# Charrrrrlie/X-as-Supervision

Hardware: AMD Instinct MI355X
Metric: images/sec HM36_Multi_SurS1 256px bs32 (full disc+gen training step) (higher is better)
Workload: dtype f32 (f16x3 split: every fp32 operand as two fp16 pieces, three products; f32 accumulate); 1 GPU; HM36_Multi_SurS1; batch_per_gpu=32, cameras=4, image=256x256, parallelism=dp1, ranks=1, precision=f16x3, dedupe=False, full=False

## Files before the change

include/xas_hip.h:

```cpp
#ifndef XAS_HIP_H
#define XAS_HIP_H

#include <stddef.h>
#include <stdint.h>

#ifdef __cplusplus
extern "C" {
#endif

const char* xas_last_error(void);
enum {
  XAS_TUNE_WGRAD_SPLIT_XCD = 1,
  XAS_TUNE_PLAIN_KLOOP = 32,
  XAS_TUNE_GLOBAL_LOAD = 64,
  XAS_TUNE_WGRAD_GLOBAL_LOAD = 128,
  XAS_TUNE_WGRAD_ALT_ORDER = 8192,
  XAS_TUNE_WGRAD_PLAIN_KLOOP = 524288,
  XAS_TUNE_SLAB_SHIFT = 15,
  XAS_TUNE_SLAB_MASK = 3,
  XAS_TUNE_SLAB_512 = 32768,
  XAS_TUNE_SLAB_128 = 65536,
  XAS_TUNE_SLAB_64 = 98304,
  XAS_TUNE_COL_REDUCE_LEAN = 262144,
  XAS_TUNE_GENERAL_KERNELS = 1 << 22,
  XAS_TUNE_NO_WIDE_TILES = 1 << 23,
  XAS_TUNE_NO_STEM_WGRAD = 1 << 24,
  XAS_TUNE_STEM_FWD_F32 = 1 << 25,
  XAS_TUNE_NO_X6P = 1 << 26,
  XAS_TUNE_X6P_ANY_K = 1 << 27
};
int xas_set_tuning(int flags);
enum { XAS_PREC_F32 = 0, XAS_PREC_BF16 = 1, XAS_PREC_BF16X6 = 2, XAS_PREC_F16X3 = 3 };
#define XAS_AMAX_SUB 32
#define XAS_AMAX_STRIDE 32
#define XAS_AMAX_SLOT_FLOATS (XAS_AMAX_SUB * XAS_AMAX_STRIDE)
enum { XAS_GRAD_IS_X = 0x100 };
int xas_set_precision(int mode);
int xas_get_precision(void);
int xas_abi_version(void);

#define XAS_HEAD_STATS 16
size_t xas_head_workspace_floats(int B, int K, int D);
int xas_head_softargmax_fwd(const float* logits, int B, int K, int D, int num_hypo, int neighbor,
                            float* kps, int64_t* z_idx, float* depth_prob_map, int groups, float* stats,
                            float* partial, void* stream);
int xas_head_softargmax_from_partials(const float* partial, int B, int K, int D, int nchunk, int num_hypo, int neighbor,
                                      float* kps, int64_t* z_idx, float* depth_prob_map, int groups, float* stats,
                                      void* stream);
int xas_head_softargmax_flip_from_partials(const float* partial, int B, int K, int D, int nchunk, int num_hypo, int neighbor,
                                           const int* perm, float* kps, int64_t* z_idx, float* depth_prob_map, int groups,
                                           void* stream);
int xas_head_softargmax_fwd_flip(const float* logits, int B, int K, int D, int num_hypo, int neighbor, const int* perm,
                                 float* kps, int64_t* z_idx, float* depth_prob_map, int groups, float* partial, void* stream);

int xas_head_softargmax_bwd(const float* logits, const float* stats, const int64_t* z_idx,
                            const float* grad_kps, int B, int K, int D, int num_hypo, int neighbor,
                            float* grad_logits, float* coef, void* stream);
int xas_head_softargmax_bwd_amax(const float* logits, const float* stats, const int64_t* z_idx,
                                 const float* grad_kps, int B, int K, int D, int num_hypo, int neighbor,
                                 float* grad_logits, float* coef, float* amax_out, void* stream);

#define XAS_HEAD_SPREAD 5
size_t xas_head_spread_workspace_floats(int B, int K, int D);
int xas_head_spread(const float* logits, int B, int K, int D, float* spread , float* workspace, void* stream);

#define XAS_GEO_NORM 1
#define XAS_GEO_MONO 2
#define XAS_GEO_PATCH 4
#define XAS_GEO_IMAGE 8
int xas_patch_to_world_fwd(const float* kps, const float* trans_image, const float* k_mat,
                           const float* pelvis, const float* rot_world, const float* trans_world,
                           int B, int Hy, int K, float image_size, float rect_width, int flags,
                           float* world, void* stream);
int xas_patch_to_world_bwd(const float* kps, const float* grad_world, const float* trans_image,
                           const float* k_mat, const float* pelvis, const float* rot_world,
                           const float* trans_world, int B, int Hy, int K, float image_size,
                           float rect_width, int flags, float* grad_kps, void* stream);

#define XAS_GEO_WORLD 16
int xas_world_to_patch_fwd(const float* pts, const float* pre_rot, float pre_scale, int pelvis_origin,
                           const float* trans_image, const float* k_mat, const float* pelvis,
                           const float* rot_world, const float* trans_world, int B, int Hy, int K,
                           float image_size, float rect_width, int flags, float* out, void* stream);
int xas_world_to_patch_bwd(const float* pts, const float* grad_out, const float* pre_rot, float pre_scale,
                           int pelvis_origin, const float* trans_image, const float* k_mat, const float* pelvis,
                           const float* rot_world, const float* trans_world, int B, int Hy, int K,
                           float image_size, float rect_width, int flags, float* grad_pts, float* grad_pre_rot,
                           void* stream);

int xas_lines_nblk(int S);
int xas_draw_lines_max_fwd(const float* kps, long kp_stride_b, long kp_stride_j, int B, int K,
                           const int* parents, const int* children, int L, unsigned fine_mask,
                           float body_width, int S, float* mask, void* stream);
int xas_draw_lines_max_bwd(const float* kps, long kp_stride_b, long kp_stride_j, int B, int K,
                           const int* parents, const int* children, int L, unsigned fine_mask,
                           float body_width, int S, const float* grad_mask, float* partial,
                           float* grad_kps_xy , void* stream);

typedef struct {
  int N, Hi, Wi, Cin;
  int Cout, R, S;
  int stride, pad;
  int Ho, Wo;
  int mode;
  const float* grad_amax;
  const float* x_amax;
} xas_conv_shape;

int xas_conv_weight_planes(const xas_conv_shape* s, int pass);
int xas_conv_kernel_class(const xas_conv_shape* s, int pass);
int xas_f16_weight_overflow(int reset);
int xas_f16_weight_overflow_peek(unsigned* device_out, void* stream);
size_t xas_split_weight_bytes(long rows, long K, int pieces);
int xas_split_weight(const float* w_packed, void* w_split, long rows, long K, int pieces, void* stream);

int xas_prepare_weights(const void* descs, int n, long blocks, void* stream);

int xas_conv_fwd(const float* x, const float* w_packed, const float* bias, float* y,
                 const xas_conv_shape* s, void* stream);

int xas_conv_fwd_head_chunks(const xas_conv_shape* s, int K, int D);
int xas_conv_fwd_head(const float* x, const float* w_packed, const float* bias, float* y, const xas_conv_shape* s,
                      int K, int D, float* head_partial, void* stream);
size_t xas_conv_fwd_bnstats_workspace_floats(const xas_conv_shape* s, int groups);
int xas_conv_fwd_bnstats(const float* x, const float* w_packed, float* y, const xas_conv_shape* s, int groups,
                         const float* pivot, float* mean, float* var_biased, long out_stride, float* count_out,
                         float* workspace, float* running_mean, float* running_var, float momentum, void* stream);
size_t xas_conv_dgrad_bn_bwd_workspace_floats(const xas_conv_shape* s, int groups);
int xas_conv_dgrad_bn_bwd(const float* dy, const float* w_packed_t, const xas_conv_shape* s, const float* xb,
                          const float* mean, const float* var_biased, const float* gamma, const float* beta, float eps,
                          int groups, double count, float* dz, float* dx, float* sums, float* workspace, float* dbeta_acc,
                          float* dgamma_acc, void* stream);
int xas_conv_dgrad(const float* dy, const float* w_packed_t, float* dx,
                   const xas_conv_shape* s, void* stream);
int xas_conv_dgrad_acc(const float* dy, const float* w_packed_t, float* dx, const xas_conv_shape* shape, void* stream);
int xas_conv_dgrad_acc_masked(const float* dy, const float* w_packed_t, float* dx, const xas_conv_shape* s,
                              const float* dprev, const uint8_t* mask, void* stream);
enum {
  XAS_PLAN_ROUTE = 0,
  XAS_PLAN_KERNEL = 1,
  XAS_PLAN_BM = 2,
  XAS_PLAN_BN = 3,
  XAS_PLAN_PIPELINED = 4,
  XAS_PLAN_PHASES = 5,
  XAS_PLAN_PIECES = 6,
  XAS_PLAN_PATCH_WIDTH = 7,
  XAS_PLAN_TPB = 8,
  XAS_PLAN_IMAGES = 9,
  XAS_PLAN_INTS = 10
};
enum { XAS_ROUTE_STEM_F16 = 1, XAS_ROUTE_STEM_F32 = 2, XAS_ROUTE_THIN_VEC_TO_SCALAR = 3, XAS_ROUTE_THIN_SCALAR_TO_VEC = 4,
       XAS_ROUTE_DIRECT = 5, XAS_ROUTE_MFMA = 6 };
enum { XAS_KERNEL_IGEMM_BUF = 1, XAS_KERNEL_IGEMM = 2, XAS_KERNEL_IGEMM_X6 = 3, XAS_KERNEL_IGEMM_X6T = 4, XAS_KERNEL_IGEMM_X6P = 5 };
int xas_conv_igemm_plan(const xas_conv_shape* s, int pass, int has_bias, int* out);
size_t xas_conv_wgrad_workspace_floats(const xas_conv_shape* s);
int xas_conv_wgrad(const float* x, const float* dy, float* dw_packed, float* workspace,
                   const xas_conv_shape* s, void* stream);
int xas_conv_wgrad_oihw(const float* x, const float* dy, float* dw_oihw, float* workspace,
                        const xas_conv_shape* s, void* stream);
int xas_conv_wgrad_acc(const float* x, const float* dy, float* dw_oihw, float* workspace,
                       const xas_conv_shape* s, void* stream);
int xas_pack_weight(const float* oihw, float* packed, int Cout, int Cin, int R, int S,
                    int transposed, void* stream);
int xas_unpack_weight(const float* packed, float* oihw, int Cout, int Cin, int R, int S,
                      int transposed, void* stream);

size_t xas_bn_workspace_floats(long M, int C, int groups);
int xas_bn_stats(const float* x, long M, int C, int groups, float* mean, float* var_biased, long out_stride,
                 float* count_out, float* workspace, float* running_mean, float* running_var, float momentum,
                 long count, void* stream);
int xas_bn_stats_from_partials(const float* partial, long rows, int C, int groups, long rows_per_group,
                               const float* pivot, float* mean, float* var_biased, long out_stride, float* count_out,
                               float* workspace, float* running_mean, float* running_var, float momentum, void* stream);
int xas_bn_bwd_sums_from_partials(const float* partial, long rows, int C, int groups, float* sums, float* workspace,
                                  float* dbeta_acc, float* dgamma_acc, void* stream);
int xas_bn_sync_merge(const float* gathered, int world, int groups, int C, long msg_stride, float* mean,
                      float* var_biased, float* running_mean, float* running_var, float momentum, void* stream);
int xas_col_sum(const float* x, long M, int C, float* out, float* workspace, void* stream);
int xas_col_sum_acc(const float* x, long M, int C, float* acc, float* workspace, void* stream);
int xas_bn_apply(const float* x, const float* mean, const float* var_biased, const float* gamma,
                 const float* beta, const float* residual, float eps, int act, long M, int C, int groups,
                 float* y, uint8_t* mask_out, void* stream);
int xas_bn_apply_amax(const float* x, const float* mean, const float* var_biased, const float* gamma,
                      const float* beta, const float* residual, float eps, int act, long M, int C, int groups,
                      float* y, uint8_t* mask_out, float* amax_out, void* stream);
int xas_abs_max(const float* x, long n, float* amax_out, void* stream);
int xas_bn_update_running(const float* mean, const float* var_biased, float* running_mean,
                          float* running_var, float momentum, long count, int C, int groups, void* stream);
int xas_bn_bwd_reduce(const float* x, const float* y, const float* dy, const float* mean,
                      const float* var_biased, const float* gamma, const float* beta, float eps, int act,
// ... 130 lines not shown
```

x-as-supervision_amd/csrc/bn.hip:

```cpp
#include "common.h"

namespace xas {


struct ColGeom { int TX, TY, CB, ncb, nslab, G; long rows_per_slab, Mg; };

static int col_geom(long M, int C, int G, ColGeom* g) {
  XAS_REQUIRE(M > 0 && C >= 4 && C % 4 == 0, "column reduce: channel count %d must be a positive multiple of 4", C);
  XAS_REQUIRE(G >= 1 && G <= 64 && M % G == 0, "column reduce: %ld rows do not split into %d equal groups", M, G);
  int cb = 4;
  while (cb < 64 && C % (cb * 2) == 0) cb *= 2;
  g->CB = cb; g->G = G; g->Mg = M / G;
  g->TX = g->CB / 4; g->TY = 256 / g->TX; g->ncb = C / g->CB;
  static const long kWant[4] = {256, 512, 128, 64};
  long want = kWant[(tune_flags() >> XAS_TUNE_SLAB_SHIFT) & XAS_TUNE_SLAB_MASK] * (G > 1 ? 2 : 1) / ((long)g->ncb * G);
  long maxslab = cdiv(g->Mg, (long)g->TY * 8);
  if (want > maxslab) want = maxslab;
  if (want < 1) want = 1;
  g->rows_per_slab = cdiv(g->Mg, want);
  g->nslab = (int)cdiv(g->Mg, g->rows_per_slab);
  return 0;
}

constexpr int kTicketWords = 65536;
// ... 687 lines not shown
      const int wo = e / C4, c = (e - wo * C4) * 4;
      float4 best = make_float4(-INFINITY, -INFINITY, -INFINITY, -INFINITY);
      int b0 = 0, b1 = 0, b2 = 0, b3 = 0;
      bool first = true;
#pragma unroll
      for (int r = 0; r < 3; ++r) {
        const int hi = ho * 2 - 1 + r;
        if ((unsigned)hi >= (unsigned)H) continue;
#pragma unroll
        for (int s = 0; s < 3; ++s) {
          const int wi = wo * 2 - 1 + s;
          if ((unsigned)wi >= (unsigned)W) continue;
          const float4 v = *reinterpret_cast<const float4*>(xn + ((size_t)hi * W + wi) * C + c);
          const int tap = r * 3 + s;
          if (first || v.x > best.x) { best.x = v.x; b0 = tap; }
          if (first || v.y > best.y) { best.y = v.y; b1 = tap; }
          if (first || v.z > best.z) { best.z = v.z; b2 = tap; }
          if (first || v.w > best.w) { best.w = v.w; b3 = tap; }
          first = false;
        }
      }
      *reinterpret_cast<float4*>(y + (obase + e) * 4) = best;
      *reinterpret_cast<char4*>(idx + (obase + e) * 4) = make_char4((char)b0, (char)b1, (char)b2, (char)b3);
    }
  }
}

__global__ __launch_bounds__(256) void maxpool_bwd_kernel(const float* __restrict__ dy, const int8_t* __restrict__ idx, int N, int H,
                                                          int W, int C, int Ho, int Wo, float* __restrict__ dx) {
  const int C4 = C / 4, per_row = W * C4;
  for (int row = blockIdx.x; row < N * H; row += gridDim.x) {
    const int n = row / H, hi = row - n * H;
    const size_t obase = (size_t)row * per_row;
    for (int e = threadIdx.x; e < per_row; e += blockDim.x) {
      const int wi = e / C4, c = (e - wi * C4) * 4;
      float4 acc = make_float4(0, 0, 0, 0);
      for (int ho = hi / 2; ho <= (hi + 1) / 2; ++ho) {
        if (ho >= Ho) continue;
        const int r = hi - (ho * 2 - 1);
        if (r < 0 || r > 2) continue;
        for (int wo = wi / 2; wo <= (wi + 1) / 2; ++wo) {
          if (wo >= Wo) continue;
          const int s = wi - (wo * 2 - 1);
          if (s < 0 || s > 2) continue;
          const size_t o = (((size_t)n * Ho + ho) * Wo + wo) * C + c;
          const char4 k = *reinterpret_cast<const char4*>(idx + o);
          const float4 g = *reinterpret_cast<const float4*>(dy + o);
          const int tap = r * 3 + s;
          if (k.x == tap) acc.x += g.x;
          if (k.y == tap) acc.y += g.y;
          if (k.z == tap) acc.z += g.z;
          if (k.w == tap) acc.w += g.w;
        }
      }
      stream_store(reinterpret_cast<float4*>(dx) + obase + e, acc);
    }
  }
}

__device__ __forceinline__ unsigned xcd_contiguous(unsigned b, unsigned nblk) {
  const unsigned per = (nblk + 7u) >> 3;
  return (b & 7u) * per + (b >> 3);
}

__global__ __launch_bounds__(256) void upsample2x_fwd_kernel(const float* __restrict__ x, int N, int H, int W, int C,
                                                             float* __restrict__ y, unsigned segs, unsigned nblk) {
  const unsigned C4 = (unsigned)C / 4, Ho = 2u * H, Wo = 2u * W;
  const unsigned bid = xcd_contiguous(blockIdx.x, nblk);
  if (bid >= nblk) return;
  const unsigned row = bid / segs, seg = bid - row * segs;
  const unsigned n = row / Ho, ho = row - n * Ho;
  const unsigned e = seg * 256u + threadIdx.x;
  if (e >= Wo * C4) return;
  const unsigned wo = e / C4, c = (e - wo * C4) * 4u;
  const float sh = fmaxf(0.f, (ho + 0.5f) * 0.5f - 0.5f), sw = fmaxf(0.f, (wo + 0.5f) * 0.5f - 0.5f);
  const int h0 = (int)sh, w0 = (int)sw;
  const int h1 = min(h0 + 1, H - 1), w1 = min(w0 + 1, W - 1);
  const float lh = sh - h0, lw = sw - w0;
  const float* base = x + (size_t)n * H * W * C + c;
  const float4 a = *reinterpret_cast<const float4*>(base + ((size_t)h0 * W + w0) * C);
  const float4 b = *reinterpret_cast<const float4*>(base + ((size_t)h0 * W + w1) * C);
  const float4 cc = *reinterpret_cast<const float4*>(base + ((size_t)h1 * W + w0) * C);
  const float4 d = *reinterpret_cast<const float4*>(base + ((size_t)h1 * W + w1) * C);
  const float h0l = 1.f - lh, w0l = 1.f - lw;
  float4 o;
  o.x = h0l * (w0l * a.x + lw * b.x) + lh * (w0l * cc.x + lw * d.x);
  o.y = h0l * (w0l * a.y + lw * b.y) + lh * (w0l * cc.y + lw * d.y);
  o.z = h0l * (w0l * a.z + lw * b.z) + lh * (w0l * cc.z + lw * d.z);
  o.w = h0l * (w0l * a.w + lw * b.w) + lh * (w0l * cc.w + lw * d.w);
  stream_store(reinterpret_cast<float4*>(y + ((size_t)row * Wo + wo) * C + c), o);
}

__global__ __launch_bounds__(256) void upsample2x_bwd_kernel(const float* __restrict__ dy, int N, int H, int W, int C,
                                                             float* __restrict__ dx, unsigned segs, unsigned nblk) {
  const unsigned C4 = (unsigned)C / 4;
  const int Ho = 2 * H, Wo = 2 * W;
  const unsigned bid = xcd_contiguous(blockIdx.x, nblk);
  if (bid >= nblk) return;
  const unsigned row = bid / segs, seg = bid - row * segs;
  const unsigned n = row / (unsigned)H;
  const int hi = (int)(row - n * (unsigned)H);
  const unsigned e = seg * 256u + threadIdx.x;
  if (e >= (unsigned)W * C4) return;
  const int wi = (int)(e / C4);
  const unsigned c = (e - (unsigned)wi * C4) * 4u;
  const float wh[4] = {hi >= 1 ? 0.25f : 0.f, hi == 0 ? 1.f : 0.75f, hi == H - 1 ? 1.f : 0.75f, hi <= H - 2 ? 0.25f : 0.f};
  const float ww[4] = {wi >= 1 ? 0.25f : 0.f, wi == 0 ? 1.f : 0.75f, wi == W - 1 ? 1.f : 0.75f, wi <= W - 2 ? 0.25f : 0.f};
  const float* base = dy + (size_t)n * Ho * Wo * C + c;
  float4 g[4][4];
#pragma unroll
  for (int k = 0; k < 4; ++k) {
    const int r = min(max(2 * hi - 1 + k, 0), Ho - 1);
#pragma unroll
    for (int l = 0; l < 4; ++l) {
      const int q = min(max(2 * wi - 1 + l, 0), Wo - 1);
      g[k][l] = *reinterpret_cast<const float4*>(base + ((size_t)r * Wo + q) * C);
    }
  }
  float4 acc = make_float4(0, 0, 0, 0);
#pragma unroll
  for (int k = 0; k < 4; ++k) {
    float4 tr = make_float4(0, 0, 0, 0);
#pragma unroll
    for (int l = 0; l < 4; ++l) {
      tr.x = fmaf(ww[l], g[k][l].x, tr.x); tr.y = fmaf(ww[l], g[k][l].y, tr.y);
      tr.z = fmaf(ww[l], g[k][l].z, tr.z); tr.w = fmaf(ww[l], g[k][l].w, tr.w);
    }
    acc.x = fmaf(wh[k], tr.x, acc.x); acc.y = fmaf(wh[k], tr.y, acc.y);
    acc.z = fmaf(wh[k], tr.z, acc.z); acc.w = fmaf(wh[k], tr.w, acc.w);
  }
  stream_store(reinterpret_cast<float4*>(dx + ((size_t)row * W + wi) * C + c), acc);
}

__global__ void sigmoid_fwd_kernel(const float* __restrict__ x, long n, float* __restrict__ y) {
  for (long i = (long)blockIdx.x * blockDim.x + threadIdx.x; i < n; i += (long)gridDim.x * blockDim.x)
    y[i] = 1.f / (1.f + __expf(-x[i]));
}
__global__ void sigmoid_bwd_kernel(const float* __restrict__ y, const float* __restrict__ dy, long n, float* __restrict__ dx) {
  for (long i = (long)blockIdx.x * blockDim.x + threadIdx.x; i < n; i += (long)gridDim.x * blockDim.x)
    dx[i] = dy[i] * y[i] * (1.f - y[i]);
}

__global__ void nchw_to_nhwc_kernel(const float* __restrict__ x, int N, int C, int HW, float* __restrict__ y, int inverse) {
  const long total = (long)N * C * HW;
  for (long i = (long)blockIdx.x * blockDim.x + threadIdx.x; i < total; i += (long)gridDim.x * blockDim.x) {
    const int c = i % C; const long t = i / C; const long p = t % HW; const long n = t / HW;
    const long j = (n * C + c) * HW + p;
    if (inverse) y[j] = x[i]; else y[i] = x[j];
  }
}

static inline unsigned ew_grid(long n, int per_block = 256) {
  long b = cdiv(n, per_block);
  return (unsigned)(b > 4096 ? 4096 : (b < 1 ? 1 : b));
}

}

using namespace xas;

extern "C" size_t xas_bn_workspace_floats(long M, int C, int groups) {
  ColGeom g;
  if (col_geom(M, C, groups, &g)) return 0;
  return (size_t)g.G * g.nslab * 2 * C + C;
}

#ifndef XAS_EW_CAP
#define XAS_EW_CAP 8192
#endif
static inline unsigned ew_grid_g(long n_per_group, int groups) {
  long b = cdiv(n_per_group, 256);
  const long cap = groups > 1 ? cdiv(XAS_EW_CAP, groups) : XAS_EW_CAP;
// ... 403 lines not shown
```

x-as-supervision_amd/csrc/common.h:

```cpp
#pragma once
#include <hip/hip_runtime.h>
#include <stdint.h>
#include <stdio.h>

#include "xas_hip.h"

namespace xas {

void set_error(const char* fmt, ...);
int tune_flags();

#define XAS_REQUIRE(cond, ...)        \
  do {                                \
    if (!(cond)) {                    \
      ::xas::set_error(__VA_ARGS__);  \
      return 1;                       \
    }                                 \
  } while (0)

#define XAS_LAUNCH_CHECK()                                               \
  do {                                                                   \
    hipError_t e_ = hipGetLastError();                                   \
    if (e_ != hipSuccess) {                                              \
      ::xas::set_error("%s:%d launch failed: %s", __FILE__, __LINE__,    \
                       hipGetErrorString(e_));                           \
      return 2;                                                          \
    }                                                                    \
  } while (0)

constexpr int kWave = 64;

__device__ __forceinline__ float wave_sum(float v) {
#pragma unroll
  for (int o = 32; o > 0; o >>= 1) v += __shfl_xor(v, o, 64);
  return v;
}
__device__ __forceinline__ float wave_max(float v) {
#pragma unroll
  for (int o = 32; o > 0; o >>= 1) v = fmaxf(v, __shfl_xor(v, o, 64));
  return v;
}

__device__ __forceinline__ float block_sum(float v, float* smem ) {
  v = wave_sum(v);
  const int lane = threadIdx.x & 63, wid = threadIdx.x >> 6, nw = (blockDim.x + 63) >> 6;
  __syncthreads();
  if (lane == 0) smem[wid] = v;
  __syncthreads();
  float r = (lane < nw) ? smem[lane] : 0.f;
  r = wave_sum(r);
  return r;
}

__device__ __forceinline__ float bn_affine(float x, float m, float rs_g, float b) {
  return __fmaf_rn(__fsub_rn(x, m), rs_g, b);
}

__device__ __forceinline__ void stream_store(float4* p, float4 v) {
#ifndef XAS_NO_NT_STORES
  typedef float f32x4_nt_t __attribute__((ext_vector_type(4)));
  __builtin_nontemporal_store(f32x4_nt_t{v.x, v.y, v.z, v.w}, reinterpret_cast<f32x4_nt_t*>(p));
#else
  *p = v;
#endif
}

__device__ __forceinline__ float4 stream_load(const float4* p) {
#ifndef XAS_NO_NT_LOADS
  typedef float f32x4_ntl_t __attribute__((ext_vector_type(4)));
  const f32x4_ntl_t v = __builtin_nontemporal_load(reinterpret_cast<const f32x4_ntl_t*>(p));
  return make_float4(v.x, v.y, v.z, v.w);
#else
  return *p;
#endif
}

constexpr int kAmaxSub = XAS_AMAX_SUB, kAmaxStride = XAS_AMAX_STRIDE;
static_assert(kAmaxSub == 32 && kAmaxSub * kAmaxStride == XAS_AMAX_SLOT_FLOATS, "amax slot layout");

__device__ __forceinline__ void publish_amax(float* out, float v) {
  __shared__ float s_amx[16];
#pragma unroll
  for (int o = 32; o > 0; o >>= 1) v = fmaxf(v, __shfl_xor(v, o, 64));
  const int nw = ((int)blockDim.x + 63) >> 6;
  if ((threadIdx.x & 63) == 0) s_amx[threadIdx.x >> 6] = v;
  __syncthreads();
  if (threadIdx.x == 0) {
    for (int w = 1; w < nw; ++w) v = fmaxf(v, s_amx[w]);
    const unsigned sub = (blockIdx.x + blockIdx.y * gridDim.x) % (unsigned)kAmaxSub;
    if (v > 0.f) atomicMax(reinterpret_cast<unsigned*>(out + sub * kAmaxStride), __float_as_uint(v));
  }
}
__device__ __forceinline__ float amax4(float a, float4 o) {
  return fmaxf(fmaxf(a, fmaxf(fabsf(o.x), fabsf(o.y))), fmaxf(fabsf(o.z), fabsf(o.w)));
}
__device__ __forceinline__ float read_amax(const float* amax) {
  float v = amax[(threadIdx.x & (kAmaxSub - 1)) * kAmaxStride];
#pragma unroll
  for (int o = 16; o > 0; o >>= 1) v = fmaxf(v, __shfl_xor(v, o, 64));
  return v;
}

static inline hipStream_t as_stream(void* s) { return reinterpret_cast<hipStream_t>(s); }
static inline long cdiv(long a, long b) { return (a + b - 1) / b; }

}
```

x-as-supervision_amd/csrc/conv.hip:

```cpp
#include <type_traits>

#include "conv_shared.h"

namespace xas {

__device__ __constant__ float4 g_zero16[4] = {{0.f, 0.f, 0.f, 0.f}, {0.f, 0.f, 0.f, 0.f}, {0.f, 0.f, 0.f, 0.f}, {0.f, 0.f, 0.f, 0.f}};

static int g_tune = 0;
int tune_flags() { return g_tune; }

__device__ __forceinline__ float4 keep_if(bool ok, float4 v) {
  v.x = ok ? v.x : 0.f; v.y = ok ? v.y : 0.f; v.z = ok ? v.z : 0.f; v.w = ok ? v.w : 0.f;
  return v;
}

template <int BM, int BN>
__device__ __forceinline__ void frag_load(const float* __restrict__ As, const float* __restrict__ Bs, int kk, int wm, int wn,
                                          int lane, float4 (&a)[TileCfg<BM, BN>::MI], float4 (&b)[TileCfg<BM, BN>::NI]) {
  using C = TileCfg<BM, BN>;
  const int i = lane & 31, h = lane >> 5;
#pragma unroll
  for (int mi = 0; mi < C::MI; ++mi)
    a[mi] = *reinterpret_cast<const float4*>(As + (wm * C::WM + mi * 32 + i) * LDK + kk * 8 + h * 4);
#pragma unroll
// ... 1436 lines not shown
  r->bm = s->Cout >= 96 ? 128 : (s->Cout > 32 ? 64 : 32);
  r->bn = (KK <= 64 && r->bm != 32) ? 64 : 128;
  const long nct = cdiv(s->Cout, r->bm), tiles = nct * cdiv(KK, r->bn);
  long sp = cdiv(split ? XAS_WGRAD_XTARGET : 1024, tiles);
  const long maxsp = M / (split ? 128 : 256);
  if (sp > maxsp) sp = maxsp;
  if (sp < 1) sp = 1;
  if (split && sp >= 8) sp -= sp % 8;
  else if (split || !(g_tune & XAS_TUNE_WGRAD_ALT_ORDER))
    while (sp > 1 && (sp * nct) % 8 != 0 && (sp * nct) > 8) --sp;
  const long per = cdiv(cdiv(M, sp), WBK) * WBK;
  r->m_per_split = (int)per;
  r->splits = (int)cdiv(M, per);
}

static WgradRoute wgrad_route(const xas_conv_shape* s, bool x_aligned) {
  if (thin_channels(s)) return {WgradKernel::Thin};
  if (s->Cout == 1) return {WgradKernel::Cout1};
  if (stem_wgrad_ok(s) && !(g_tune & XAS_TUNE_NO_STEM_WGRAD)) return {WgradKernel::Stem};
  WgradRoute r{};
  r.vec = x_aligned && s->Cin % 4 == 0;
  const bool buf = r.vec && wgrad_offsets_fit(s) && !(g_tune & XAS_TUNE_WGRAD_GLOBAL_LOAD);
  if (buf && precision_of(s) != XAS_PREC_F32 && s->Cout % 4 == 0 && s->Cout >= 16) {
    if (!(g_tune & XAS_TUNE_GENERAL_KERNELS) && wgrad_x6t_plan(s, &r.bm, &r.splits, &r.m_per_split)) r.kernel = WgradKernel::SplitTap;
    else { r.kernel = WgradKernel::Split; wgrad_plan(s, true, &r); }
  } else {
    r.kernel = buf && s->Cin % 32 == 0 ? WgradKernel::F32Buf : WgradKernel::F32Global;
    wgrad_plan(s, false, &r);
  }
  return r;
}

extern "C" int xas_set_tuning(int flags) { g_tune = flags; return 0; }
extern "C" int xas_set_precision(int mode) {
  XAS_REQUIRE(mode >= 0 && mode <= 3, "set_precision: 0 = exact fp32 MFMA, 1 = bf16 MFMA (not fp32 accurate), 2 = bf16x6 (fp32-accurate, no "
              "operand maxima needed), 3 = f16x3 (default; fp32-accurate; launches that come without the maxima of their operands run as bf16x6)");
  g_precision = mode;
  return 0;
}
extern "C" int xas_get_precision(void) { return g_precision; }

namespace xas {
__global__ void stem_overflow_peek_kernel(unsigned* out) { if (g_f16_weight_overflow_stem) atomicOr(out, 1u); }
int stem_weight_overflow_peek(unsigned* device_out, void* stream) {
  hipLaunchKernelGGL(stem_overflow_peek_kernel, dim3(1), dim3(1), 0, as_stream(stream), device_out);
  XAS_LAUNCH_CHECK();
  return 0;
}
int stem_weight_overflow(int reset) {
  unsigned v = 0u;
  if (hipMemcpyFromSymbol(&v, HIP_SYMBOL(g_f16_weight_overflow_stem), sizeof(v)) != hipSuccess) return -1;
  if (v && reset) {
    const unsigned z = 0u;
    (void)hipMemcpyToSymbol(HIP_SYMBOL(g_f16_weight_overflow_stem), &z, sizeof(z));
  }
  return v ? 1 : 0;
}
}

static IgemmParams fwd_problem(const xas_conv_shape* s) {
  IgemmParams p{};
  p.N = s->N; p.a_amax = s->grad_amax;
  p.Hs = s->Hi; p.Ws = s->Wi; p.Cs = s->Cin; p.Hd = s->Ho; p.Wd = s->Wo; p.Cd = s->Cout;
  p.R = s->R; p.S = s->S; p.stride = s->stride; p.pad = s->pad; p.Hrow = s->Ho; p.Wrow = s->Wo; p.tune = g_tune;
  p.div_hw.init((unsigned)(s->Ho * s->Wo)); p.div_w.init((unsigned)s->Wo);
  p.src_elems = (long)p.N * p.Hs * p.Ws * p.Cs; p.wgt_elems = (long)p.Cd * p.R * p.S * p.Cs;
  return p;
}
static IgemmParams dgrad_problem(const xas_conv_shape* s) {
  IgemmParams p{};
  p.N = s->N; p.a_amax = s->grad_amax;
  p.Hs = s->Ho; p.Ws = s->Wo; p.Cs = s->Cout; p.Hd = s->Hi; p.Wd = s->Wi; p.Cd = s->Cin;
  p.R = s->R; p.S = s->S; p.stride = s->stride; p.pad = s->pad; p.tune = g_tune;
  p.src_elems = (long)p.N * p.Hs * p.Ws * p.Cs; p.wgt_elems = (long)p.Cd * p.R * p.S * p.Cs;
  return p;
}
struct IgemmGrid { int Mrows_max, phases; };
static IgemmGrid fwd_grid(const xas_conv_shape* s) { return {s->N * s->Ho * s->Wo, 1}; }
static IgemmGrid dgrad_grid(const xas_conv_shape* s) {
  const int Hp = (s->Hi + s->stride - 1) / s->stride, Wp = (s->Wi + s->stride - 1) / s->stride;
  return {s->N * Hp * Wp, s->stride * s->stride};
}

static int fwd_stats_tile_rows(const xas_conv_shape* s, int groups) {
  if (!s || groups < 1) return 0;
  if (fwd_route(s, false) != FwdRoute::Mfma || s->Cout % 4 != 0) return 0;
  if (fwd_images_per_launch(s) < s->N || s->N % groups) return 0;
  const long M = (long)s->N * s->Ho * s->Wo, Mg = M / groups;
  const int prec = precision_of(s);
  int bm, bn;
  if (prec == XAS_PREC_F32) pick_tile(s->Cout, M, 1, &bm, &bn);
  else bm = pick_tile_x6(fwd_problem(s), 0, (int)M, 1, planes_of(prec, 0, has_amax_for(s, 0))).bm;
  if (Mg % bm) return 0;
  if ((M / bm) * 2 * (long)s->Cout * 4 >= 0x7fffff00l) return 0;
  return bm;
}

static int launch_thin(bool vec_to_scalar, const xas_conv_shape* s, const float* src, const float* w, const float* bias,
                       float* out, int flip, hipStream_t st) {
  const int C = thin_channels(s);
  const ThinParams tp = thin_params(s->N, s->Hi, s->Wi, C, s->pad, flip);
  const dim3 grid(thin_grid((long)s->N * s->Hi * s->Wi, C));
  if (vec_to_scalar) hipLaunchKernelGGL(thin_vec2scalar_kernel, grid, dim3(256), 0, st, src, w, bias, out, tp);
  else hipLaunchKernelGGL(thin_scalar2vec_kernel, grid, dim3(256), 0, st, src, w, bias, out, tp);
  XAS_LAUNCH_CHECK();
  return 0;
}

static int conv_fwd_impl(const float* x, const float* w_packed, const float* bias, float* y, const xas_conv_shape* s,
                         void* stream, float* stat_partial, const float* stat_pivot, float* head_partial = nullptr) {
  if (check_shape(s, "conv_fwd") || check_fwd_dims(s, "conv_fwd")) return 1;
  XAS_REQUIRE(x && w_packed && y, "conv_fwd: null buffer");
  const long xi = (long)s->Hi * s->Wi * s->Cin, yi = (long)s->Ho * s->Wo * s->Cout;
  const int per = fwd_images_per_launch(s);
  if (per < s->N) {
    XAS_REQUIRE(!stat_partial, "conv_fwd: the statistics epilogue needs a single launch");
    return for_image_ranges(s, per, [&](int n0, const xas_conv_shape* part) {
      float* hp = head_partial ? head_partial + (size_t)n0 * (s->Ho * s->Wo / 64) * (s->Cout / 64) * 67 : nullptr;
      return conv_fwd_impl(x + (size_t)n0 * xi, w_packed, bias, y + (size_t)n0 * yi, part, stream, nullptr, nullptr, hp);
    });
  }
  hipStream_t st = as_stream(stream);
  const FwdRoute route = fwd_route(s, bias != nullptr);
  switch (route) {
    case FwdRoute::StemF16:
    case FwdRoute::StemF32: {
      const int tiles = (int)(cdiv(s->Ho, ST_TH) * cdiv(s->Wo, ST_TW));
      if (route == FwdRoute::StemF16)
        hipLaunchKernelGGL(stem_fwd_f16_kernel, dim3((unsigned)cdiv(tiles, STH_TPB), s->N), dim3(256), 0, st, x, w_packed, y, s->N, s->Hi,
                           s->Wi, s->Ho, s->Wo, s->grad_amax);
      else
        hipLaunchKernelGGL(stem_fwd_kernel, dim3((unsigned)cdiv(tiles, ST_TPB), s->N), dim3(256), 0, st, x, w_packed, y, s->N, s->Hi,
                           s->Wi, s->Ho, s->Wo);
      XAS_LAUNCH_CHECK();
      return 0;
    }
    case FwdRoute::ThinVecToScalar: return launch_thin(true, s, x, w_packed, bias, y, 0, st);
    case FwdRoute::ThinScalarToVec: return launch_thin(false, s, x, w_packed, bias, y, 0, st);
    case FwdRoute::Direct: {
      const long total = (long)s->N * s->Ho * s->Wo * s->Cout;
      hipLaunchKernelGGL(direct_fwd_kernel, dim3((unsigned)cdiv(total, 256)), dim3(256), 0, st, x, w_packed, bias, y, *s);
      XAS_LAUNCH_CHECK();
      return 0;
    }
    case FwdRoute::Mfma: break;
  }
  XAS_REQUIRE((((uintptr_t)x | (uintptr_t)w_packed) & 15) == 0, "conv_fwd: operands must be 16-byte aligned");
  IgemmParams p = fwd_problem(s);
  p.src = x; p.wgt = w_packed; p.bias = bias; p.out = y;
  p.stat_partial = stat_partial; p.stat_pivot = stat_pivot;
  p.head_partial = head_partial;
  const IgemmGrid g = fwd_grid(s);
  return dispatch_igemm<0>(p, precision_of(s), g.Mrows_max, g.phases, st);
}

extern "C" int xas_conv_fwd(const float* x, const float* w_packed, const float* bias, float* y,
                            const xas_conv_shape* s, void* stream) {
  return conv_fwd_impl(x, w_packed, bias, y, s, stream, nullptr, nullptr);
}

extern "C" int xas_conv_fwd_head_chunks(const xas_conv_shape* s, int K, int D) {
  if (!s || K < 1 || D != 64) return 0;
  if (s->R != 1 || s->S != 1 || s->stride != 1 || s->pad != 0 || s->Wo != 64 || (s->Ho * s->Wo) % 64 != 0) return 0;
  if (s->Cout != K * D || fwd_route(s, false) != FwdRoute::Mfma || precision_of(s) == XAS_PREC_F32) return 0;
  return s->Ho * s->Wo / 64;
}

extern "C" int xas_conv_fwd_head(const float* x, const float* w_packed, const float* bias, float* y, const xas_conv_shape* s,
                                 int K, int D, float* head_partial, void* stream) {
  XAS_REQUIRE(head_partial && xas_conv_fwd_head_chunks(s, K, D) > 0, "conv_fwd_head: shape not taken (xas_conv_fwd_head_chunks) or null buffer");
  return conv_fwd_impl(x, w_packed, bias, y, s, stream, nullptr, nullptr, head_partial);
}

extern "C" int xas_conv_weight_planes(const xas_conv_shape* s, int pass) {
  if (!s) return 0;
  const int prec = precision_of(s);
  if (prec == XAS_PREC_F32) return 0;
  const bool mfma = pass == 0 ? fwd_route(s, false) == FwdRoute::Mfma : dgrad_route(s) == DgradRoute::Mfma;
  return mfma ? planes_of(prec, pass, has_amax_for(s, pass)) : 0;
}

extern "C" int xas_conv_kernel_class(const xas_conv_shape* s, int pass) {
  if (!s) return 0;
  const int prec = precision_of(s);
  const int split = prec == XAS_PREC_F32 ? 1 : (prec == XAS_PREC_BF16 ? 2 : (planes_of(prec, pass, has_amax_for(s, pass)) == 2 ? 4 : 3));
  if (pass == 0) {
    const FwdRoute f = fwd_route(s, false);
    return f == FwdRoute::StemF16 ? 4 : f == FwdRoute::StemF32 ? 1 : f == FwdRoute::Mfma ? split : 0;
  }
  if (pass == 1) return dgrad_route(s) == DgradRoute::Mfma ? split : 0;
  xas_conv_shape part = *s;
  part.N = images_per_launch(s->N, (long)s->Hi * s->Wi * s->Cin, (long)s->Ho * s->Wo * s->Cout);
  const WgradKernel k = wgrad_route(&part, true).kernel;
  if (k == WgradKernel::Thin || k == WgradKernel::Cout1) return 0;
  return (k == WgradKernel::SplitTap || k == WgradKernel::Split) ? split : 1;
}

static size_t epilogue_workspace_floats(long M, int C, int groups, int bm) {
  if (!bm) return xas_bn_workspace_floats(M, C, groups);
  return (size_t)(M / bm) * 2 * C + xas_bn_workspace_floats(M / bm, 2 * C, groups);
}
extern "C" size_t xas_conv_fwd_bnstats_workspace_floats(const xas_conv_shape* s, int groups) {
  if (!s || groups < 1) return 0;
  return epilogue_workspace_floats((long)s->N * s->Ho * s->Wo, s->Cout, groups, fwd_stats_tile_rows(s, groups));
}

extern "C" int xas_conv_fwd_bnstats(const float* x, const float* w_packed, float* y, const xas_conv_shape* s, int groups,
                                    const float* pivot, float* mean, float* var_biased, long out_stride, float* count_out,
                                    float* workspace, float* running_mean, float* running_var, float momentum,
                                    void* stream) {
  XAS_REQUIRE(s && groups >= 1 && s->N % groups == 0, "conv_fwd_bnstats: the batch does not split into %d groups", groups);
  XAS_REQUIRE(workspace && mean && var_biased, "conv_fwd_bnstats: null buffer");
  const long M = (long)s->N * s->Ho * s->Wo, Mg = M / groups;
  const int bm = fwd_stats_tile_rows(s, groups);
  if (!bm) {
    const int rc = conv_fwd_impl(x, w_packed, nullptr, y, s, stream, nullptr, nullptr);
    if (rc) return rc;
    return xas_bn_stats(y, M, s->Cout, groups, mean, var_biased, out_stride, count_out, workspace, running_mean,
                        running_var, momentum, Mg, stream);
  }
  const long rows = M / bm;
  const int rc = conv_fwd_impl(x, w_packed, nullptr, y, s, stream, workspace, pivot);
  if (rc) return rc;
  return xas_bn_stats_from_partials(workspace, rows, s->Cout, groups, Mg, pivot, mean, var_biased, out_stride, count_out,
                                    workspace + (size_t)rows * 2 * s->Cout, running_mean, running_var, momentum, stream);
}

static int conv_dgrad_impl(const float* dy, const float* w_packed_t, float* dx, const xas_conv_shape* s, void* stream,
                           int accumulate, const float* acc_src = nullptr, const unsigned char* acc_mask = nullptr,
                           const IgemmParams* bnb = nullptr) {
  if (check_shape(s, "conv_dgrad")) return 1;
  const DgradRoute route = dgrad_route(s);
  XAS_REQUIRE(!accumulate || (route == DgradRoute::Mfma && s->Cin % 4 == 0),
              "conv_dgrad_acc: only the MFMA path accumulates (Cout %% 32 == 0, Cin %% 4 == 0, Cin >= 16)");
// ... 158 lines not shown
extern "C" size_t xas_conv_wgrad_workspace_floats(const xas_conv_shape* s) {
  if (!s) return 0;
  const WgradKernel k = wgrad_route(s, true).kernel;
  if (k == WgradKernel::Thin) return (size_t)(cdiv((long)s->N * s->Hi * s->Wi, kThinChunk) + 1) * thin_channels(s) * 9;
  if (k == WgradKernel::Cout1) return (size_t)cdiv((long)s->N * s->Ho * s->Wo, kCout1Chunk) * s->R * s->S * s->Cin;
  if (stem_wgrad_ok(s)) return (size_t)2 * kStemWgradBlocks * ST_CO * ST_K;
  WgradRoute f32{}, split{}, tap{};
  wgrad_plan(s, false, &f32);
  wgrad_plan(s, true, &split);
  wgrad_x6t_plan(s, &tap.bm, &tap.splits, &tap.m_per_split);
  int sp = f32.splits > split.splits ? f32.splits : split.splits;
  if (tap.splits > sp) sp = tap.splits;
  return (size_t)sp * s->Cout * s->R * s->S * s->Cin;
}

template <int BM, int BN, bool VEC>
static int launch_wgrad(const WgradParams& p, int splits, hipStream_t st) {
  const size_t lds = (size_t)2 * WBK * ((BM + 4) + (BN + 4)) * sizeof(float);
  static bool attr_set_dev[kMaxDevices] = {};
  bool& attr_set = attr_set_dev[current_device()];
  if (!attr_set) {
    (void)hipFuncSetAttribute(reinterpret_cast<const void*>(&wgrad_kernel<BM, BN, VEC>),
                        hipFuncAttributeMaxDynamicSharedMemorySize, (int)lds);
    attr_set = true;
  }
  WgradParams q = p;
  q.nct = (int)cdiv(p.Cout, BM);
  q.ntiles = q.nct * (int)cdiv(p.KK, BN);
  q.nsplits = splits;
  q.tune = g_tune;
  dim3 grid((unsigned)(8 * cdiv(splits, 8) * q.ntiles));
  hipLaunchKernelGGL((wgrad_kernel<BM, BN, VEC>), grid, dim3(256), lds, st, q);
  XAS_LAUNCH_CHECK();
  return 0;
}

template <int BM, int BN, int T, bool PIPE = true>
static int launch_wgrad_buf_t(const WgradParams& p, int splits, hipStream_t st) {
  if (PIPE && (g_tune & XAS_TUNE_WGRAD_PLAIN_KLOOP)) return launch_wgrad_buf_t<BM, BN, T, false>(p, splits, st);
  size_t lds = (size_t)2 * WBK * ((BM + 4) + (BN + 32)) * sizeof(float);
  static size_t attr_set_dev[kMaxDevices] = {};
  size_t& attr_set = attr_set_dev[current_device()];
  if (attr_set < lds) {
    (void)hipFuncSetAttribute(reinterpret_cast<const void*>(&wgrad_buf_kernel<BM, BN, T, PIPE>),
                        hipFuncAttributeMaxDynamicSharedMemorySize, (int)lds);
    attr_set = lds;
  }
  WgradParams q = p;
  q.nct = (int)cdiv(p.Cout, BM);
  q.ntiles = q.nct * (int)cdiv(p.KK, BN);
  q.nsplits = splits;
  q.tune = g_tune;
  dim3 grid((unsigned)((g_tune & XAS_TUNE_WGRAD_ALT_ORDER) ? splits * q.ntiles : 8 * cdiv((long)splits * q.nct, 8) * (q.ntiles / q.nct)));
  hipLaunchKernelGGL((wgrad_buf_kernel<BM, BN, T, PIPE>), grid, dim3(256), lds, st, q);
  XAS_LAUNCH_CHECK();
  return 0;
}

template <int BM, int BN>
static int launch_wgrad_buf(const WgradParams& p, int splits, hipStream_t st) {
  if (p.Cin % BN == 0) return launch_wgrad_buf_t<BM, BN, 1>(p, splits, st);
  if (p.Cin % (BN / 2) == 0) return launch_wgrad_buf_t<BM, BN, 2>(p, splits, st);
  if constexpr (BN >= 128) {
    if (p.Cin % (BN / 4) == 0) return launch_wgrad_buf_t<BM, BN, 4>(p, splits, st);
  }
  set_error("wgrad_buf: Cin=%d does not divide into tap groups of a %d-column tile", p.Cin, BN);
  return 1;
}

template <int V> using IntC = std::integral_constant<int, V>;
template <class F>
static int with_wgrad_tile(int bm, int bn, F&& f) {
  if (bm == 32) return f(IntC<32>(), IntC<128>());
  if (bn == 64) return bm == 128 ? f(IntC<128>(), IntC<64>()) : f(IntC<64>(), IntC<64>());
  return bm == 128 ? f(IntC<128>(), IntC<128>()) : f(IntC<64>(), IntC<128>());
}

static int conv_wgrad_impl(const float* x, const float* dy, float* dw_packed, float* workspace, const xas_conv_shape* s,
                           void* stream, bool oihw, bool accumulate = false) {
  const int rflag = (oihw ? 1 : 0) | (accumulate ? 2 : 0);
  if (check_shape(s, "conv_wgrad")) return 1;
  XAS_REQUIRE(x && dy && dw_packed && workspace, "conv_wgrad: null buffer");
  XAS_REQUIRE(s->Cout % 4 == 0 || s->Cout == 1, "conv_wgrad: Cout=%d must be a multiple of 4 (or 1)", s->Cout);
  const long xi = (long)s->Hi * s->Wi * s->Cin, yi = (long)s->Ho * s->Wo * s->Cout;
  const int per = images_per_launch(s->N, xi, yi);
  if (per < s->N && (oihw || accumulate))
    return for_image_ranges(s, per, [&](int n0, const xas_conv_shape* part) {
      return conv_wgrad_impl(x + (size_t)n0 * xi, dy + (size_t)n0 * yi, dw_packed, workspace, part, stream, oihw, accumulate || n0 > 0);
    });
  hipStream_t st = as_stream(stream);
  const WgradRoute r = wgrad_route(s, ((uintptr_t)x & 15) == 0);
  switch (r.kernel) {
    case WgradKernel::Thin: {
      const bool cout1 = s->Cout == 1;
      const int C = cout1 ? s->Cin : s->Cout;
      const ThinParams tp = thin_params(s->N, s->Hi, s->Wi, C, s->pad, 0);
      const long M = (long)s->N * s->Hi * s->Wi;
      int chunks = (int)cdiv(M, kThinChunk);
      if (chunks > 1024) chunks = 1024;
      const int per_chunk = (int)(cdiv(cdiv(M, chunks), 256) * 256);
      chunks = (int)cdiv(M, per_chunk);
      hipLaunchKernelGGL(thin_wgrad_kernel, dim3(chunks), dim3(256), 0, st, cout1 ? dy : x, cout1 ? x : dy, workspace, tp,
                         cout1 ? -1 : 1, per_chunk);
      XAS_LAUNCH_CHECK();
      const long n = (long)C * 9;
      if (oihw || !cout1) {
        hipLaunchKernelGGL(slab_reduce_kernel2, dim3((unsigned)cdiv(n, 64)), dim3(slab_threads()), 0, st, workspace, chunks, n,
                           accumulate ? 2 : 0, 1, 1, 1, dw_packed);
      } else {
        hipLaunchKernelGGL(slab_reduce_kernel2, dim3((unsigned)cdiv(n, 64)), dim3(slab_threads()), 0, st, workspace, chunks, n, 0, 1, 1, 1,
                           workspace + (size_t)chunks * n);
        XAS_LAUNCH_CHECK();
        hipLaunchKernelGGL(pack_weight_kernel, dim3((unsigned)cdiv(n, 256)), dim3(256), 0, st, workspace + (size_t)chunks * n,
                           dw_packed, 1, C, 3, 3, 0, 0);
      }
      XAS_LAUNCH_CHECK();
      return 0;
    }
    case WgradKernel::Cout1: {
      const int KK = s->R * s->S * s->Cin;
      const int chunks = (int)cdiv((long)s->N * s->Ho * s->Wo, kCout1Chunk);
      hipLaunchKernelGGL(wgrad_cout1_kernel, dim3((unsigned)cdiv(KK, 64), (unsigned)chunks), dim3(64), 0, st, x, dy,
                         workspace, *s, kCout1Chunk);
      XAS_LAUNCH_CHECK();
      hipLaunchKernelGGL(slab_reduce_kernel2, dim3((unsigned)cdiv(KK, 64)), dim3(slab_threads()), 0, st, workspace, chunks, (long)KK,
                         rflag, s->Cin, s->R, s->S, dw_packed);
      XAS_LAUNCH_CHECK();
      return 0;
    }
    case WgradKernel::Stem: {
      const int patches = s->N * (s->Ho / ST_TH) * (s->Wo / ST_TW);
      const int ppb = (int)cdiv(patches, kStemWgradBlocks), blocks = (int)cdiv(patches, ppb);
      hipLaunchKernelGGL(stem_wgrad_kernel, dim3((unsigned)blocks), dim3(256), 0, st, x, dy, workspace, s->N, s->Hi, s->Wi,
                         s->Ho, s->Wo, patches, ppb);
      XAS_LAUNCH_CHECK();
      const long n = (long)ST_CO * ST_K;
      hipLaunchKernelGGL(slab_reduce_kernel2, dim3((unsigned)cdiv(n, 64)), dim3(slab_threads()), 0, st, workspace, 2 * blocks, n,
                         rflag, s->Cin, s->R, s->S, dw_packed);
      XAS_LAUNCH_CHECK();
      return 0;
    }
    default: break;
  }
  const int splits = r.splits;
  WgradParams p{};
  p.x = x; p.dy = dy; p.out = (splits == 1 && !oihw) ? dw_packed : workspace;
  p.a_amax = (s->mode & XAS_GRAD_IS_X) ? s->x_amax : s->grad_amax;
  p.b_amax = (s->mode & XAS_GRAD_IS_X) ? s->grad_amax : s->x_amax;
  p.N = s->N; p.Hi = s->Hi; p.Wi = s->Wi; p.Cin = s->Cin; p.Cout = s->Cout; p.R = s->R; p.S = s->S;
  p.stride = s->stride; p.pad = s->pad; p.Ho = s->Ho; p.Wo = s->Wo;
  p.KK = s->R * s->S * s->Cin; p.M = s->N * s->Ho * s->Wo; p.m_per_split = r.m_per_split;
  p.div_hw.init((unsigned)(s->Ho * s->Wo)); p.div_w.init((unsigned)s->Wo);
  p.div_cin.init((unsigned)s->Cin); p.div_s.init((unsigned)s->S);
  const int pieces = planes_of(precision_of(s), 2, has_amax_for(s, 2));
  int rc;
  switch (r.kernel) {
    case WgradKernel::SplitTap: rc = launch_wgrad_x6t(p, r.bm, splits, r.m_per_split, pieces, st); break;
    case WgradKernel::Split: rc = launch_wgrad_x6(p, r.bm, r.bn, splits, pieces, st); break;
    case WgradKernel::F32Buf:
      rc = with_wgrad_tile(r.bm, r.bn, [&](auto bm, auto bn) { return launch_wgrad_buf<decltype(bm)::value, decltype(bn)::value>(p, splits, st); });
      break;
    default:
      rc = with_wgrad_tile(r.bm, r.bn, [&](auto bm, auto bn) {
        constexpr int BM = decltype(bm)::value, BN = decltype(bn)::value;
        return r.vec ? launch_wgrad<BM, BN, true>(p, splits, st) : launch_wgrad<BM, 128, false>(p, splits, st);
      });
  }
  if (rc) return rc;
  const long n = (long)s->Cout * p.KK;
  if (oihw || splits > 1) {
    hipLaunchKernelGGL(slab_reduce_kernel2, dim3((unsigned)cdiv(n, 64)), dim3(slab_threads()), 0, st, workspace, splits, n,
                       rflag, s->Cin, s->R, s->S, dw_packed);
    XAS_LAUNCH_CHECK();
  }
  return 0;
}

extern "C" int xas_conv_wgrad(const float* x, const float* dy, float* dw_packed, float* workspace,
                              const xas_conv_shape* s, void* stream) {
  return conv_wgrad_impl(x, dy, dw_packed, workspace, s, stream, false);
}

extern "C" int xas_conv_wgrad_oihw(const float* x, const float* dy, float* dw_oihw, float* workspace,
                                   const xas_conv_shape* s, void* stream) {
  return conv_wgrad_impl(x, dy, dw_oihw, workspace, s, stream, true);
}

extern "C" int xas_conv_wgrad_acc(const float* x, const float* dy, float* dw_oihw, float* workspace,
                                  const xas_conv_shape* s, void* stream) {
  return conv_wgrad_impl(x, dy, dw_oihw, workspace, s, stream, true, true);
}

extern "C" int xas_pack_weight(const float* oihw, float* packed, int Cout, int Cin, int R, int S, int transposed,
                               void* stream) {
  XAS_REQUIRE(oihw && packed && Cout > 0 && Cin > 0 && R > 0 && S > 0, "pack_weight: bad arguments");
  const long total = (long)Cout * Cin * R * S;
  hipLaunchKernelGGL(pack_weight_kernel, dim3((unsigned)cdiv(total, 256)), dim3(256), 0, as_stream(stream), oihw, packed,
                     Cout, Cin, R, S, transposed, 0);
  XAS_LAUNCH_CHECK();
  return 0;
}

extern "C" int xas_unpack_weight(const float* packed, float* oihw, int Cout, int Cin, int R, int S, int transposed,
                                 void* stream) {
  XAS_REQUIRE(oihw && packed && Cout > 0 && Cin > 0 && R > 0 && S > 0, "unpack_weight: bad arguments");
  const long total = (long)Cout * Cin * R * S;
  hipLaunchKernelGGL(pack_weight_kernel, dim3((unsigned)cdiv(total, 256)), dim3(256), 0, as_stream(stream), packed, oihw,
                     Cout, Cin, R, S, transposed, 1);
  XAS_LAUNCH_CHECK();
  return 0;
}
```

x-as-supervision_amd/csrc/conv_shared.h:

```cpp
#pragma once
#include "common.h"

namespace xas {

using f32x16 = __attribute__((ext_vector_type(16))) float;

constexpr int BK = 32;
constexpr int LDK = BK + 4;

struct FastDiv {
  unsigned d, mul, shift;
  __host__ void init(unsigned dd) {
    d = dd;
    if (dd == 1) { mul = 0; shift = 0; return; }
    unsigned s = 0;
    while ((1ull << s) < dd) ++s;
    unsigned long long m = ((1ull << (31 + s)) + dd - 1) / dd;
    mul = (unsigned)m; shift = s;
  }
  __device__ __forceinline__ unsigned div(unsigned n) const {
    return d == 1 ? n : (unsigned)(((unsigned long long)n * mul) >> (31 + shift));
  }
};

struct IgemmParams {
  const float* src;
  const float* wgt;
  const float* bias;
  float* out;
  int N;
  int Hs, Ws, Cs;
  int Hd, Wd, Cd;
  int R, S, stride, pad;
  FastDiv div_hw, div_w;
  int Hrow, Wrow;
  int tune;
  int nMt, nNt, mt_per_xcd;
  int t2d_tw;
  int tpb;
  int xn, nt_per_x;
  long src_elems, wgt_elems;
  int accumulate;
  const float* acc_src;
  const unsigned char* acc_mask;
  float* stat_partial;
  const float* stat_pivot;
  const float* bnb_x;
  const float* bnb_mean; const float* bnb_var; const float* bnb_gamma; const float* bnb_beta;
  float bnb_eps;
  int bnb_rows_per_group;
  float* bnb_partial;
  const float* a_amax;
  float* head_partial;
};

constexpr int kMaxDevices = 16;
static inline int current_device() {
  int d = 0;
  if (hipGetDevice(&d) != hipSuccess || d < 0 || d >= kMaxDevices) d = 0;
  return d;
}

template <int BM, int BN>
struct TileCfg {
  static constexpr int WAVES_M = (BM == 64 && BN == 256) ? 1 : (BM >= 64 && BN >= 64) ? 2 : (BM < 64 ? 1 : 4);
  static constexpr int WAVES_N = 4 / WAVES_M;
  static constexpr int WM = BM / WAVES_M, WN = BN / WAVES_N;
  static constexpr int MI = WM / 32, NI = WN / 32;
  static_assert(MI >= 1 && NI >= 1, "tile too small");
};

typedef unsigned int u32x4 __attribute__((ext_vector_type(4)));
constexpr unsigned kOOB = 0x80000000u;

__device__ __forceinline__ float4 buf_load16(__amdgpu_buffer_rsrc_t r, unsigned voff, unsigned soff) {
  const u32x4 v = __builtin_amdgcn_raw_buffer_load_b128(r, (int)voff, (int)soff, 0);
  return make_float4(__uint_as_float(v.x), __uint_as_float(v.y), __uint_as_float(v.z), __uint_as_float(v.w));
}

typedef __bf16 bf16x8_t __attribute__((ext_vector_type(8)));
typedef __bf16 bf16x2_t __attribute__((ext_vector_type(2)));
typedef float f32x2_t __attribute__((ext_vector_type(2)));
constexpr int LDKH = BK + 8;

__device__ __forceinline__ uint2 pack_bf16x4(float4 v) {
  const bf16x2_t lo = __builtin_convertvector(f32x2_t{v.x, v.y}, bf16x2_t);
  const bf16x2_t hi = __builtin_convertvector(f32x2_t{v.z, v.w}, bf16x2_t);
  return make_uint2(__builtin_bit_cast(unsigned, lo), __builtin_bit_cast(unsigned, hi));
}

__device__ __forceinline__ float4 sub_bf16x4(float4 v, uint2 q) {
  return make_float4(v.x - __uint_as_float(q.x << 16), v.y - __uint_as_float(q.x & 0xffff0000u),
                     v.z - __uint_as_float(q.y << 16), v.w - __uint_as_float(q.y & 0xffff0000u));
}

typedef _Float16 f16x2_t __attribute__((ext_vector_type(2)));
typedef _Float16 f16x8_t __attribute__((ext_vector_type(8)));
constexpr float kF16WScale = 1024.f;
constexpr float kF16AScale = 16.f;
int stem_weight_overflow(int reset);
int stem_weight_overflow_peek(unsigned* device_out, void* stream);
constexpr float kF16Descale = 1.f / (kF16WScale * kF16AScale);
__device__ __forceinline__ float f16_grad_scale(const float* amax, float* inv) {
  const unsigned bits = __builtin_amdgcn_readfirstlane(__float_as_uint(read_amax(amax)));
  const int e = (int)((bits >> 23) & 0xffu);
  if (e < 40 || e > 250) { *inv = 1.f; return 1.f; }
  *inv = __uint_as_float((unsigned)(e - 14) << 23);
  return __uint_as_float((unsigned)(268 - e) << 23);
}

__device__ __forceinline__ uint2 pack_f16x4(float4 v) {
  const f16x2_t lo = {(_Float16)v.x, (_Float16)v.y}, hi = {(_Float16)v.z, (_Float16)v.w};
  return make_uint2(__builtin_bit_cast(unsigned, lo), __builtin_bit_cast(unsigned, hi));
}
__device__ __forceinline__ float4 sub_f16x4(float4 v, uint2 q) {
  const f16x2_t lo = __builtin_bit_cast(f16x2_t, q.x), hi = __builtin_bit_cast(f16x2_t, q.y);
  return make_float4(v.x - (float)lo.x, v.y - (float)lo.y, v.z - (float)hi.x, v.w - (float)hi.y);
}
__device__ __forceinline__ void split_f16x4(float4 v, float s, uint2& h1, uint2& h2) {
  unsigned a, b, c, d;
  asm("v_fma_mixlo_f16 %0, %2, %3, 0\n\t"
      "v_fma_mixlo_f16 %1, %2, %5, 0\n\t"
      "v_fma_mixhi_f16 %0, %2, %4, 0\n\t"
      "v_fma_mixhi_f16 %1, %2, %6, 0"
      : "=&v"(a), "=&v"(b) : "v"(s), "v"(v.x), "v"(v.y), "v"(v.z), "v"(v.w));
  asm("v_fma_mixlo_f16 %0, %2, %3, -%7 op_sel_hi:[0,0,1]\n\t"
      "v_fma_mixlo_f16 %1, %2, %5, -%8 op_sel_hi:[0,0,1]\n\t"
      "v_fma_mixhi_f16 %0, %2, %4, -%7 op_sel:[0,0,1] op_sel_hi:[0,0,1]\n\t"
      "v_fma_mixhi_f16 %1, %2, %6, -%8 op_sel:[0,0,1] op_sel_hi:[0,0,1]"
      : "=&v"(c), "=&v"(d) : "v"(s), "v"(v.x), "v"(v.y), "v"(v.z), "v"(v.w), "v"(a), "v"(b));
  h1 = make_uint2(a, b);
  h2 = make_uint2(c, d);
}
template <int P> struct Pieces { uint2 q[P]; };
template <int P> __device__ __forceinline__ Pieces<P> split_pieces(float4 r, float s);
template <int P> __device__ __forceinline__ uint2 pack_piece4(float4 v) { return P == 2 ? pack_f16x4(v) : pack_bf16x4(v); }
// ... 235 lines not shown
          const float4 o = prevv[j];
          const unsigned mb = pmask[j];
          v.x += (mb & 1u) ? o.x : 0.f; v.y += (mb & 2u) ? o.y : 0.f;
          v.z += (mb & 4u) ? o.z : 0.f; v.w += (mb & 8u) ? o.w : 0.f;
        }
        stream_store(reinterpret_cast<float4*>(p.out + orow * p.Cd + nn), v);
      }
    }
    if constexpr (HEAD && MODE == 0 && BM == 64 && BNH == 64) {
      if (p.head_partial != nullptr && nh0 < p.Cd) {
        const int tid = threadIdx.x;
        const int c = tid & 63, part = tid >> 6;
        const float bc = p.bias ? p.bias[nh0 + c] : 0.f;
        float v[16];
        float mx = -INFINITY;
#pragma unroll
        for (int j = 0; j < 16; ++j) { v[j] = lds[(part + 4 * j) * LDT + c] + bc; mx = fmaxf(mx, v[j]); }
#pragma unroll
        for (int o = 32; o > 0; o >>= 1) mx = fmaxf(mx, __shfl_xor(mx, o, 64));
        float* red = lds + BM * LDT;
        if (c == 0) red[part] = mx;
        __syncthreads();
        const float Mx = fmaxf(fmaxf(red[0], red[1]), fmaxf(red[2], red[3]));
        float z = 0.f, sx = 0.f;
#pragma unroll
        for (int j = 0; j < 16; ++j) {
          const float e = __expf(v[j] - Mx);
          z += e;
          sx = fmaf(e, (float)(part + 4 * j), sx);
        }
        red[8 + part * 64 + c] = z;
        float zs = z;
#pragma unroll
        for (int o = 32; o > 0; o >>= 1) { zs += __shfl_xor(zs, o, 64); sx += __shfl_xor(sx, o, 64); }
        if (c == 0) { red[264 + part] = zs; red[268 + part] = sx; }
        __syncthreads();
        const int img = m0 / HW, pix0 = m0 - img * HW;
        float* rec = p.head_partial + (((size_t)img * (HW >> 6) + (pix0 >> 6)) * (p.Cd >> 6) + (nh0 >> 6)) * 67;
        if (part == 0) rec[3 + c] = (red[8 + c] + red[8 + 64 + c]) + (red[8 + 128 + c] + red[8 + 192 + c]);
        if (tid == 64) {
          const float tot = (red[264] + red[265]) + (red[266] + red[267]);
          rec[0] = Mx;
          rec[1] = (red[268] + red[269]) + (red[270] + red[271]);
          rec[2] = tot * (float)(pix0 >> 6);
        }
      }
    }
    if (MODE == 0 && want_stats) {
      constexpr int PARTS = 256 / BNH;
      const int tid = threadIdx.x;
      const int c = tid % BNH, part = tid / BNH;
      const int n = nh0 + c;
      const float pv = (p.stat_pivot && n < p.Cd) ? p.stat_pivot[n] : 0.f;
      float s = 0.f, q = 0.f;
#pragma unroll 8
      for (int r = part; r < BM; r += PARTS) {
        const float v = lds[r * LDT + c] - pv;
        s += v; q = fmaf(v, v, q);
      }
      float* red = lds + BM * LDT;
      red[(part * BNH + c) * 2] = s; red[(part * BNH + c) * 2 + 1] = q;
      __syncthreads();
      if (part == 0 && n < p.Cd) {
#pragma unroll
        for (int k = 1; k < PARTS; ++k) { s += red[(k * BNH + c) * 2]; q += red[(k * BNH + c) * 2 + 1]; }
        *reinterpret_cast<float2*>(p.stat_partial + ((size_t)(m0 / BM) * p.Cd + n) * 2) = make_float2(s, q);
      }
    }
  }
}


struct WgradParams {
  const float* x; const float* dy; float* out;
  int N, Hi, Wi, Cin, Cout, R, S, stride, pad, Ho, Wo;
  int KK;
  int M;
  int m_per_split;
  int nct, ntiles, nsplits;
  int tune;
  int t2d_tw, pps;
  const float* a_amax; const float* b_amax;
  FastDiv div_hw, div_w, div_cin, div_s;
};

constexpr int WBK = 32;

static inline bool tap_tile_ok(int R, int S, int stride, int pad, int Hs, int Ws, int Hd, int Wd, int Cs, int N) {
  if (R != 3 || S != 3 || stride != 1 || pad != 1 || Hd != Hs || Wd != Ws || Cs % 32 != 0 || Hd % 8 != 0) return false;
  return Wd % 16 == 0 || (Wd == 8 && N % 2 == 0);
}
static inline int tap_patch_width(int Wd) { return Wd % 16 == 0 ? 16 : 8; }

#ifndef XAS_TILE128_MIN_BLOCKS
#define XAS_TILE128_MIN_BLOCKS 256
#endif
static inline void pick_tile(int Cd, long Mrows_max, int phases, int* bm, int* bn, bool wide = false) {
  if (Cd >= 96) {
    const long blocks128 = cdiv(Mrows_max, 128) * cdiv(Cd, 128) * phases;
    if (blocks128 <= XAS_TILE128_MIN_BLOCKS) { *bm = 64; *bn = 64; }
    else if (wide && Cd % 256 == 0) { *bm = 64; *bn = 256; }
    else { *bm = 128; *bn = 128; }
  } else if (Cd >= 48) { *bm = 128; *bn = 64; }
  else { *bm = 128; *bn = 32; }
}

int launch_igemm_x6(const IgemmParams& p, int mode, int Mrows_max, int phases, int pieces, hipStream_t st);
struct X6Tile {
  int bm, bn;
  enum Kernel { General, Tap, Persistent } kernel;
};
X6Tile pick_tile_x6(const IgemmParams& p, int mode, int Mrows_max, int phases, int pieces);
int x6p_tiles_per_block(const IgemmParams& p, int Mrows_max);
int launch_wgrad_x6(const WgradParams& p, int bm, int bn, int splits, int pieces, hipStream_t st);
bool wgrad_x6t_plan(const xas_conv_shape* s, int* bm, int* splits, int* pps);
int launch_wgrad_x6t(const WgradParams& p, int bm, int splits, int pps, int pieces, hipStream_t st);

}
```

x-as-supervision_amd/csrc/conv_x6.hip:

```cpp
#include <type_traits>

#include "conv_shared.h"

namespace xas {

typedef short s16x4_t __attribute__((ext_vector_type(4)));
typedef short s16x8_t __attribute__((ext_vector_type(8)));

constexpr int XH = 16;
constexpr int XLDH = XH;
__device__ __forceinline__ int xswz(int row, int half) { return (half ^ ((row >> 3) & 1)) << 3; }


__device__ __forceinline__ void zero_acc(f32x16& a) {
#pragma unroll
  for (int e = 0; e < 16; ++e) a[e] = 0.f;
}
template <class T, int N>
__device__ __forceinline__ void zero_acc(T (&a)[N]) {
#pragma unroll
  for (int n = 0; n < N; ++n) zero_acc(a[n]);
}
template <int P, int MI, int NI>
__device__ __forceinline__ void scale_acc(f32x16 (&acc)[MI][NI], float desc) {
// ... 29 lines not shown

__device__ __forceinline__ void xcd_tile(const IgemmParams& p, int& mt, int& nt) {
  const int xcd = blockIdx.x & 7, qb = blockIdx.x >> 3;
  const int xi = xcd / p.xn, xj = xcd - xi * p.xn;
  const int ml = qb / p.nt_per_x;
  mt = xi * p.mt_per_xcd + ml;
  nt = xj * p.nt_per_x + (qb - ml * p.nt_per_x);
}

template <int P, int NI>
struct WeightFrags {
  __amdgpu_buffer_rsrc_t rsrc;
  unsigned blk_bytes, voff, nblk0;
  __device__ __forceinline__ WeightFrags(const IgemmParams& p, int Ktot, int nblk, int lane) {
    blk_bytes = (unsigned)(Ktot / 16) * P * 1024u;
    const long wbytes = (long)((p.Cd + 31) / 32) * blk_bytes;
    rsrc = __builtin_amdgcn_make_buffer_rsrc(const_cast<float*>(p.wgt), 0, (int)wbytes, 0x00020000);
    voff = (unsigned)lane * 16u;
    nblk0 = (unsigned)nblk;
  }
  __device__ __forceinline__ void load(uint4 (&gb)[P][NI], unsigned hc) const {
#pragma unroll
    for (int ni = 0; ni < NI; ++ni)
#pragma unroll
      for (int pc = 0; pc < P; ++pc)
        gb[pc][ni] = __builtin_bit_cast(uint4, __builtin_amdgcn_raw_buffer_load_b128(
            rsrc, (int)voff, (int)((nblk0 + ni) * blk_bytes + (hc * P + pc) * 1024u), 0));
  }
};

template <int P, bool B_FIRST, int MI, int NI>
__device__ __forceinline__ void mfma_products(f32x16 (&acc)[MI][NI], const uint4 (&fa)[P][MI], const uint4 (&fb)[P][NI]) {
#pragma unroll
  for (int t = 0; t < Products<P>::N; ++t)
#pragma unroll
    for (int mi = 0; mi < MI; ++mi)
#pragma unroll
      for (int ni = 0; ni < NI; ++ni) {
        const uint4 a = fa[Products<P>::A[t]][mi], b = fb[Products<P>::B[t]][ni];
        acc[mi][ni] = B_FIRST ? mfma_piece<P>(b, a, acc[mi][ni]) : mfma_piece<P>(a, b, acc[mi][ni]);
      }
}

template <int BM, int P, int MI>
__device__ __forceinline__ void read_plane_frags(uint4 (&fa)[P][MI], const unsigned short* sb, int row0, int i, int hh) {
#pragma unroll
  for (int pc = P - 1; pc >= 0; --pc)
#pragma unroll
    for (int mi = 0; mi < MI; ++mi)
      fa[pc][mi] = *reinterpret_cast<const uint4*>(sb + pc * (BM * XLDH) + (row0 + mi * 32 + i) * XLDH + xswz(i, hh));
}

typedef s16x4_t __attribute__((address_space(3))) * lds_s16x4_p;
__device__ __forceinline__ uint4 tr_frag(const unsigned char* base, unsigned off, int row_stride) {
  const s16x4_t lo = __builtin_amdgcn_ds_read_tr16_b64_v4i16((lds_s16x4_p)(base + off));
  const s16x4_t hi = __builtin_amdgcn_ds_read_tr16_b64_v4i16((lds_s16x4_p)(base + off + 4 * row_stride));
  return __builtin_bit_cast(uint4, __builtin_shufflevector(lo, hi, 0, 1, 2, 3, 4, 5, 6, 7));
}

struct PatchGeom {
  int H, W, tw, tws, tn_cnt, hw, npix_img, npix, tiles_x, per_img;
  __device__ __forceinline__ PatchGeom(int t2d_tw, int H_, int W_) {
    H = H_; W = W_;
    tw = t2d_tw; tws = tw == 16 ? 4 : 3;
    tn_cnt = 128 >> (3 + tws);
    hw = tw + 2; npix_img = 10 * hw; npix = tn_cnt * npix_img;
    tiles_x = W / tw; per_img = tiles_x * (H >> 3);
  }
  __device__ __forceinline__ void origin(int patch, int& img0, int& y0, int& x0) const {
    img0 = (patch / per_img) * tn_cnt;
    const int tt = patch % per_img;
    y0 = (tt / tiles_x) * 8; x0 = (tt % tiles_x) * tw;
  }
  __device__ __forceinline__ void halo_pixel(int pix, int& tn, int& dy, int& dx) const {
    tn = pix / npix_img;
    const int pr = pix - tn * npix_img, hy = pr / hw;
    dy = hy - 1; dx = pr - hy * hw - 1;
  }
  __device__ __forceinline__ bool inside(int img, int gy, int gx, int N) const {
    return (unsigned)gy < (unsigned)H && (unsigned)gx < (unsigned)W && img < N;
  }
  __device__ __forceinline__ long pixel(int img, int gy, int gx) const { return ((long)img * H + gy) * W + gx; }
};

__device__ unsigned g_f16_weight_overflow = 0u;
__device__ __forceinline__ void f16_weight_check(float4 a, float4 b) {
  const float m = fmaxf(fmaxf(fmaxf(fabsf(a.x), fabsf(a.y)), fmaxf(fabsf(a.z), fabsf(a.w))),
                        fmaxf(fmaxf(fabsf(b.x), fabsf(b.y)), fmaxf(fabsf(b.z), fabsf(b.w))));
  if (!(m < 65504.f)) atomicOr(&g_f16_weight_overflow, 1u);
}
template <int P>
__device__ __forceinline__ void split_store_weight(float4 r0, float4 r1, unsigned short* o) {
  if (P == 2) {
    r0.x *= kF16WScale; r0.y *= kF16WScale; r0.z *= kF16WScale; r0.w *= kF16WScale;
    r1.x *= kF16WScale; r1.y *= kF16WScale; r1.z *= kF16WScale; r1.w *= kF16WScale;
    f16_weight_check(r0, r1);
  }
#pragma unroll
  for (int pc = 0; pc < P; ++pc) {
    const uint2 q0 = pack_piece4<P>(r0), q1 = pack_piece4<P>(r1);
    *reinterpret_cast<uint4*>(o + pc * 512) = make_uint4(q0.x, q0.y, q1.x, q1.y);
    if (pc + 1 < P) { r0 = sub_piece4<P>(r0, q0); r1 = sub_piece4<P>(r1, q1); }
  }
}

template <int P>
__global__ __launch_bounds__(256) void split_weight_kernel(const float* __restrict__ src, unsigned short* __restrict__ dst,
                                                           int rows, int K, long total ) {
  const long id = (long)blockIdx.x * 256 + threadIdx.x;
  if (id >= total) return;
  const int lane = (int)(id & 63);
  const long blk = id >> 6;
  const int nhc = K / 16;
  const int hc = (int)(blk % nhc), rb = (int)(blk / nhc);
  const int row = rb * 32 + (lane & 31), k0 = hc * 16 + (lane >> 5) * 8;
  float4 r0 = make_float4(0, 0, 0, 0), r1 = r0;
  if (row < rows) {
    r0 = *reinterpret_cast<const float4*>(src + (size_t)row * K + k0);
    r1 = *reinterpret_cast<const float4*>(src + (size_t)row * K + k0 + 4);
  }
  split_store_weight<P>(r0, r1, dst + (blk * P) * 512 + lane * 8);
}

#ifndef XAS_X6_WAVES2
#define XAS_X6_WAVES2 2
#endif
#ifndef XAS_X6_WAVES2_WIDE
#define XAS_X6_WAVES2_WIDE 2
#endif
#ifndef XAS_WX6_WAVES2
#define XAS_WX6_WAVES2 2
#endif
template <int BM, int BN, int MODE, int P, bool BNB = false>
__global__ __launch_bounds__(256, (P == 2 ? (BM == 64 && BN == 256 ? XAS_X6_WAVES2_WIDE : XAS_X6_WAVES2) : 2)) void igemm_x6_kernel(IgemmParams p) {
  using C = TileCfg<BM, BN>;
  constexpr int PLANE = BM * XLDH;
  constexpr int HBUF = P * PLANE;
  constexpr int AP = BM / 64;
  extern __shared__ __align__(16) float lds[];
  unsigned short* S = reinterpret_cast<unsigned short*>(lds);
  const int tid = threadIdx.x, lane = tid & 63;
  const int wave = __builtin_amdgcn_readfirstlane(tid >> 6);
  const int wm = wave / C::WAVES_N, wn = wave % C::WAVES_N;
  const int kq4 = tid & 3, arow = tid >> 2;

  int Hrow = p.Hrow, Wrow = p.Wrow;
  int ph = 0, pw = 0, base_r = 0, base_s = 0, nr = p.R, ns = p.S, off_h = -p.pad, off_w = -p.pad, rstep = 1;
  int sa = p.stride;
  if (MODE == 1) {
    const int st = p.stride;
    ph = blockIdx.z / st; pw = blockIdx.z % st;
    Hrow = (p.Hd - ph + st - 1) / st; Wrow = (p.Wd - pw + st - 1) / st;
    base_r = (ph + p.pad) % st; base_s = (pw + p.pad) % st;
    nr = base_r < p.R ? (p.R - base_r + st - 1) / st : 0;
    ns = base_s < p.S ? (p.S - base_s + st - 1) / st : 0;
    off_h = (ph + p.pad - base_r) / st; off_w = (pw + p.pad - base_s) / st;
    rstep = st; sa = 1;
  }
  const int Mrows = p.N * Hrow * Wrow;
  int mt, nt;
  xcd_tile(p, mt, nt);
  if (mt >= p.nMt || nt >= p.nNt) return;
  const int m0 = mt * BM, n0 = nt * BN;
  if (m0 >= Mrows) return;
#ifndef XAS_X6_PRIO
#define XAS_X6_PRIO 3
// ... 150 lines not shown
  const int ntl = min(p.tpb, p.nMt - mt0);
  const int n0 = nt * BN;
  const int nk = p.Cs / BK;
  const F16Scales<P> f16(p.a_amax);

  const __amdgpu_buffer_rsrc_t rsrcA = __builtin_amdgcn_make_buffer_rsrc(const_cast<float*>(p.src), 0, (int)(p.src_elems * 4), 0x00020000);
  auto voff_of = [&](int t) -> unsigned {
    const int m = (mt0 + t) * BM + arow;
    return (t < ntl && m < Mrows) ? (unsigned)(((long)m * p.Cs + kq4 * 4) * 4) : kOOB;
  };
  const WeightFrags<P, C::NI> wfr(p, p.Cs, n0 / 32 + wn * (C::WN / 32), lane);

  int a_t = 0, a_c = 0, b_c = 0;
  unsigned voffA = voff_of(0);
  float4 ra_0[2], ra_1[2];
  auto load_a = [&](float4 (&ra)[2]) {
    const unsigned soff = (unsigned)(a_c * BK) * 4u;
    ra[0] = buf_load16(rsrcA, voffA, soff);
    ra[1] = buf_load16(rsrcA, voffA, soff + XH * 4u);
    if (++a_c == nk) { a_c = 0; ++a_t; voffA = voff_of(a_t); }
  };
  auto load_b = [&](uint4 (&gb)[P][C::NI], int h) {
    wfr.load(gb, (unsigned)(b_c * (BK / 16) + h));
    if (h) { if (++b_c == nk) b_c = 0; }
  };
  auto split_store = [&](int buf, int h, const float4 (&ra)[2]) {
    const Pieces<P> pcs = split_pieces<P>(ra[h], f16.sa);
#pragma unroll
    for (int pc = 0; pc < P; ++pc)
      *reinterpret_cast<uint2*>(S + buf * HBUF + pc * PLANE + arow * XLDH + xswz(arow, kq4 >> 1) + (kq4 & 1) * 4) = pcs.q[pc];
  };
  const int i = lane & 31, hh = lane >> 5;
  f32x16 acc[C::MI][C::NI];
  auto compute = [&](int buf, const uint4 (&gb)[P][C::NI]) {
    uint4 fa[P][C::MI];
    read_plane_frags<BM>(fa, S + buf * HBUF, 0, i, hh);
    mfma_products<P, true>(acc, fa, gb);
  };
  uint4 gb_0[P][C::NI], gb_1[P][C::NI];
  load_a(ra_0);
  load_a(ra_1);
  for (int t = 0; t < ntl; ++t) {
    b_c = 0;
    load_b(gb_0, 0);
    load_b(gb_1, 1);
    zero_acc(acc);
    split_store(0, 0, ra_0);
    for (int ks = 0; ks < nk; ks += 2) {
      __syncthreads();
      compute(0, gb_0);
      load_b(gb_0, 0);
      split_store(1, 1, ra_0);
      __syncthreads();
      load_a(ra_0);
      compute(1, gb_1);
      load_b(gb_1, 1);
      split_store(0, 0, ra_1);
      __syncthreads();
      compute(0, gb_0);
      if (ks + 2 < nk) load_b(gb_0, 0);
      split_store(1, 1, ra_1);
      __syncthreads();
      load_a(ra_1);
      compute(1, gb_1);
      if (ks + 2 < nk) { load_b(gb_1, 1); split_store(0, 0, ra_0); }
    }
    scale_acc<P>(acc, f16.desc);
    f32x16 unused;
    zero_acc(unused);
    int n0v = n0, lanev = lane, wnv = wn;
    asm volatile("" : "+s"(n0v), "+v"(lanev), "+s"(wnv));
    igemm_epilogue<BM, BN, MODE, false, BN / 64, false>(p, acc, unused, (mt0 + t) * BM, n0v, 0, wnv, lanev, Mrows, HW, Wrow, 0, 0, lds);
    __syncthreads();
  }
}

constexpr int XT_PIXB = 80;
constexpr int XT_NJ = 7;
constexpr int XT_PLANE_MAX = 200 * XT_PIXB;

#ifndef XAS_X6T_WAVES
#define XAS_X6T_WAVES 2
#endif
template <int BN, int MODE, int P>
__global__ __launch_bounds__(256, XAS_X6T_WAVES) void igemm_x6t_kernel(IgemmParams p) {
  constexpr int BM = 128;
  using C = TileCfg<BM, BN>;
  extern __shared__ __align__(16) float lds[];
  unsigned char* S = reinterpret_cast<unsigned char*>(lds);
  const int tid = threadIdx.x, lane = tid & 63;
  const int wave = __builtin_amdgcn_readfirstlane(tid >> 6);
  const int wm = wave / C::WAVES_N, wn = wave % C::WAVES_N;
  const int H = p.Hd, W = p.Wd;
  const PatchGeom g(p.t2d_tw, H, W);
  const int plane_b = g.npix * XT_PIXB;

  int mt, nt;
  xcd_tile(p, mt, nt);
  if (mt >= p.nMt || nt >= p.nNt) return;
  const int m0 = mt * BM, n0 = nt * BN;
  const int Mrows = p.N * H * W;
  __builtin_amdgcn_s_setprio(XAS_X6_PRIO);
  const F16Scales<P> f16(p.a_amax);
  int img0, y0, x0;
  g.origin(mt, img0, y0, x0);
  const int cchunks = p.Cs / BK;
  const int ntap = p.R * p.S;

  const __amdgpu_buffer_rsrc_t rsrcA = __builtin_amdgcn_make_buffer_rsrc(const_cast<float*>(p.src), 0, (int)(p.src_elems * 4), 0x00020000);
  unsigned voffA[XT_NJ];
#pragma unroll
  for (int j = 0; j < XT_NJ; ++j) {
    const int item = tid + 256 * j, pix = item >> 3, q = item & 7;
    voffA[j] = kOOB;
    if (pix < g.npix) {
      int tn, dy, dx;
      g.halo_pixel(pix, tn, dy, dx);
      const int gy = y0 + dy, gx = x0 + dx, img = img0 + tn;
      if (g.inside(img, gy, gx, p.N)) voffA[j] = (unsigned)((g.pixel(img, gy, gx) * p.Cs + q * 4) * 4);
    }
  }
  float4 ra[XT_NJ];
  auto load_chunk = [&](int chunk) {
    const unsigned soff = (unsigned)(chunk * BK) * 4u;
#pragma unroll
    for (int j = 0; j < XT_NJ; ++j) ra[j] = buf_load16(rsrcA, voffA[j], soff);
  };
  auto stage = [&]() {
#pragma unroll
    for (int j = 0; j < XT_NJ; ++j) {
      const int item = tid + 256 * j, pix = item >> 3, q = item & 7;
      if (pix < g.npix) {
        const Pieces<P> pcs = split_pieces<P>(ra[j], f16.sa);
        unsigned char* d = S + pix * XT_PIXB + q * 8;
#pragma unroll
        for (int pc = 0; pc < P; ++pc) *reinterpret_cast<uint2*>(d + pc * plane_b) = pcs.q[pc];
      }
    }
  };
  const int i = lane & 31, hh = lane >> 5;
  int fbase[C::MI];
#pragma unroll
  for (int mi = 0; mi < C::MI; ++mi) {
    const int r = wm * C::WM + mi * 32 + i;
    const int tn = r >> (3 + g.tws), ty = (r >> g.tws) & 7, tx = r & (g.tw - 1);
    fbase[mi] = (tn * g.npix_img + (ty + 1) * g.hw + (tx + 1)) * XT_PIXB + hh * 16;
  }
  const WeightFrags<P, C::NI> wfr(p, ntap * p.Cs, n0 / 32 + wn * (C::WN / 32), lane);
  int b_chunk = 0, b_tap = 0;
  const int nhs = 2 * ntap * cchunks;
  int b_left = nhs;
  auto load_b = [&](uint4 (&gb)[P][C::NI], int h) {
    wfr.load(gb, (unsigned)((b_tap * p.Cs + b_chunk * BK) / 16 + h));
    if (h) {
      const bool more = b_left > 2;
      b_left -= more ? 2 : 0;
      int t2 = b_tap + 1, c2 = b_chunk;
      if (t2 == ntap) { t2 = 0; ++c2; }
      b_tap = more ? t2 : b_tap; b_chunk = more ? c2 : b_chunk;
    }
  };
  f32x16 acc[C::MI][C::NI];
  zero_acc(acc);
  f32x16 acc2;
  zero_acc(acc2);
  auto read_frag = [&](uint4 (&fa)[P][C::MI], int tapoff) {
#pragma unroll
    for (int pc = P - 1; pc >= 0; --pc)
#pragma unroll
      for (int mi = 0; mi < C::MI; ++mi)
        fa[pc][mi] = *reinterpret_cast<const uint4*>(S + pc * plane_b + fbase[mi] + tapoff);
  };
  auto tap_off = [&](int t) {
    const int jr = t / p.S, js = t - jr * p.S;
    const int dy = MODE == 0 ? jr - p.pad : p.pad - jr, dx = MODE == 0 ? js - p.pad : p.pad - js;
    return (dy * g.hw + dx) * XT_PIXB;
  };
  uint4 gb_0[P][C::NI], gb_1[P][C::NI];
  uint4 fa_0[P][C::MI], fa_1[P][C::MI];
  load_chunk(0);
  load_b(gb_0, 0);
  load_b(gb_1, 1);
  for (int chunk = 0; chunk < cchunks; ++chunk) {
    stage();
    __syncthreads();
    load_chunk(chunk + 1 < cchunks ? chunk + 1 : chunk);
    int off = tap_off(0);
    read_frag(fa_0, off);
    for (int t = 0; t < ntap; ++t) {
      read_frag(fa_1, off + 32);
      mfma_products<P, true>(acc, fa_0, gb_0);
      load_b(gb_0, 0);
      off = tap_off(t + 1 < ntap ? t + 1 : t);
      read_frag(fa_0, off);
      mfma_products<P, true>(acc, fa_1, gb_1);
      load_b(gb_1, 1);
    }
    __syncthreads();
  }
  scale_acc<P>(acc, f16.desc);
  igemm_epilogue<BM, BN, MODE, false, (BN == 128 ? 2 : 1)>(p, acc, acc2, m0, n0, wm, wn, lane, Mrows, H * W, W, 0, 0, lds);
}

template <int BN>
constexpr size_t igemm_x6t_lds(int P) {
  size_t a = (size_t)P * XT_PLANE_MAX;
  size_t b = ((size_t)128 * (BN / (BN == 128 ? 2 : 1) + 4) + 2 * 256) * sizeof(float);
  return a > b ? a : b;
}


template <int BM, int BN>
constexpr size_t igemm_x6_lds(int P, bool bnb) {
  size_t a = (size_t)2 * P * BM * XLDH * sizeof(unsigned short);
  size_t b = ((size_t)BM * (BN / (BN >= 128 ? BN / 64 : 1) + 4) + 2 * 256) * sizeof(float);
  size_t c = bnb ? ((size_t)2 * TileCfg<BM, BN>::WAVES_M * 32 * (BN + 4) + 2 * 256) * sizeof(float) : 0;
  a = a > b ? (a > c ? a : c) : (b > c ? b : c);
  return a;
}

static int pick_xcd_grid(double a_bytes, double b_bytes, int nMt, int nNt, int m_units) {
  double best = 0;
  int pick = 1;
  for (int xn = 1; xn <= 8; xn *= 2) {
    if (nNt % xn != 0 || m_units < 8 / xn) continue;
    const int xm = 8 / xn, ntx = nNt / xn, mtx = (int)cdiv(nMt, xm);
    const double slice = b_bytes / xn;
    const double rounds = slice <= 2.5e6 ? 1.0 : (double)cdiv(mtx, 64 / ntx > 0 ? 64 / ntx : 1);
    const double cost = a_bytes * xn + slice * 8 * rounds;
    if (xn == 1 || cost < best * 0.9) { best = cost; pick = xn; }
  }
  return pick;
}

template <int BM, int BN, int MODE, int P, bool BNB>
static int launch_igemm_x6_t(const IgemmParams& p, int Mrows_max, int phases, hipStream_t st) {
  constexpr size_t lds = igemm_x6_lds<BM, BN>(P, BNB);
  static bool attr_set_dev[kMaxDevices] = {};
  bool& attr_set = attr_set_dev[current_device()];
  if (!attr_set && lds > 64 * 1024) {
    (void)hipFuncSetAttribute(reinterpret_cast<const void*>(&igemm_x6_kernel<BM, BN, MODE, P, BNB>),
                              hipFuncAttributeMaxDynamicSharedMemorySize, (int)lds);
    attr_set = true;
  }
  IgemmParams q = p;
  q.nMt = (int)cdiv(Mrows_max, BM); q.nNt = (int)cdiv(p.Cd, BN);
  q.xn = pick_xcd_grid((double)Mrows_max * phases * p.Cs * 4.0 * (MODE == 0 ? p.stride * p.stride : 1),
                       (double)p.Cd * p.R * p.S * p.Cs * 2.0 * P, q.nMt, q.nNt, q.nMt);
  q.nt_per_x = q.nNt / q.xn;
  q.mt_per_xcd = (int)cdiv(q.nMt, 8 / q.xn);
  dim3 grid((unsigned)(8 * q.mt_per_xcd * q.nt_per_x), 1, (unsigned)phases);
  hipLaunchKernelGGL((igemm_x6_kernel<BM, BN, MODE, P, BNB>), grid, dim3(256), lds, st, q);
  XAS_LAUNCH_CHECK();
  return 0;
}

template <int BN, int MODE, int P>
static int launch_igemm_x6t(const IgemmParams& p, int Mrows_max, hipStream_t st) {
  constexpr size_t lds = igemm_x6t_lds<BN>(P);
  IgemmParams q = p;
  q.t2d_tw = tap_patch_width(p.Wd);
  q.nMt = Mrows_max / 128; q.nNt = (int)cdiv(p.Cd, BN);
  q.xn = 1; q.nt_per_x = q.nNt; q.mt_per_xcd = (int)cdiv(q.nMt, 8);
  dim3 grid((unsigned)(8 * q.mt_per_xcd * q.nt_per_x), 1, 1);
  hipLaunchKernelGGL((igemm_x6t_kernel<BN, MODE, P>), grid, dim3(256), lds, st, q);
  XAS_LAUNCH_CHECK();
  return 0;
}

#ifndef XAS_X6P_MAX_K
#define XAS_X6P_MAX_K 4096
#endif
static bool x6p_takes(const IgemmParams& p, int mode, int phases) {
  if (p.tune & XAS_TUNE_NO_X6P) return false;
  if (p.Cs > XAS_X6P_MAX_K && !(p.tune & XAS_TUNE_X6P_ANY_K)) return false;
  const int hr = mode == 0 ? p.Hrow : p.Hd, wr = mode == 0 ? p.Wrow : p.Wd;
  return p.R == 1 && p.S == 1 && p.stride == 1 && p.pad == 0 && phases == 1 && p.Cs % (2 * BK) == 0 && p.Hs == hr && p.Ws == wr &&
         !p.t2d_tw && !p.bnb_x && p.a_amax != nullptr && (p.Cd & 3) == 0;
}

int x6p_tiles_per_block(const IgemmParams& p, int Mrows_max) {
  const long tiles = cdiv(Mrows_max, 64) * cdiv(p.Cd, 256);
  const int tpb = (int)(tiles / (768 * 4));
  return tpb < 1 ? 1 : (tpb > 8 ? 8 : tpb);
}

template <int MODE>
static int launch_igemm_x6p(const IgemmParams& p, int Mrows_max, hipStream_t st) {
  constexpr size_t lds = igemm_x6_lds<64, 256>(2, false);
  IgemmParams q = p;
  q.nMt = (int)cdiv(Mrows_max, 64); q.nNt = (int)cdiv(p.Cd, 256);
  const int tpb = x6p_tiles_per_block(p, Mrows_max);
  q.tpb = tpb;
  const int nMg = (int)cdiv(q.nMt, tpb);
  q.xn = pick_xcd_grid((double)Mrows_max * p.Cs * 4.0, (double)p.Cd * p.Cs * 2.0 * 2, q.nMt, q.nNt, nMg);
  q.nt_per_x = q.nNt / q.xn;
  q.mt_per_xcd = (int)cdiv(nMg, 8 / q.xn);
  dim3 grid((unsigned)(8 * q.mt_per_xcd * q.nt_per_x), 1, 1);
  hipLaunchKernelGGL((igemm_x6p_kernel<MODE>), grid, dim3(256), lds, st, q);
  XAS_LAUNCH_CHECK();
  return 0;
}

template <class F>
static int with_pieces(int pieces, F&& f) {
  if (pieces == 2) return f(std::integral_constant<int, 2>());
  if (pieces == 3) return f(std::integral_constant<int, 3>());
  return f(std::integral_constant<int, 1>());
}

X6Tile pick_tile_x6(const IgemmParams& p, int mode, int Mrows_max, int phases, int pieces) {
  X6Tile t{64, 256, X6Tile::General};
  if (mode == 0 && p.head_partial) return t;
  pick_tile(p.Cd, Mrows_max, phases, &t.bm, &t.bn);
  const bool bnb = mode == 1 && pieces != 2 && p.bnb_x;
  if (!(p.tune & XAS_TUNE_GENERAL_KERNELS) && t.bm == 128 && phases == 1 && !p.bnb_x &&
      tap_tile_ok(p.R, p.S, p.stride, p.pad, p.Hs, p.Ws, p.Hd, p.Wd, p.Cs, p.N)) t.kernel = X6Tile::Tap;
  else if (!bnb && !(p.tune & XAS_TUNE_NO_WIDE_TILES)) {
    pick_tile(p.Cd, Mrows_max, phases, &t.bm, &t.bn, true);
    if (pieces == 2 && t.bn == 256 && x6p_takes(p, mode, phases)) t.kernel = X6Tile::Persistent;
  }
  return t;
}

template <int MODE, int P, bool BNB>
static int launch_igemm_x6_tile(const IgemmParams& p, const X6Tile& t, int Mrows_max, int phases, hipStream_t st) {
  if constexpr (!BNB) {
    if (t.bn == 256) return launch_igemm_x6_t<64, 256, MODE, P, false>(p, Mrows_max, phases, st);
  }
  if (t.bn == 128) return launch_igemm_x6_t<128, 128, MODE, P, BNB>(p, Mrows_max, phases, st);
  if (t.bm == 64) return launch_igemm_x6_t<64, 64, MODE, P, BNB>(p, Mrows_max, phases, st);
  if (t.bn == 64) return launch_igemm_x6_t<128, 64, MODE, P, BNB>(p, Mrows_max, phases, st);
  return launch_igemm_x6_t<128, 32, MODE, P, BNB>(p, Mrows_max, phases, st);
}

template <int MODE, int P>
static int launch_igemm_x6_p(const IgemmParams& p, int Mrows_max, int phases, hipStream_t st) {
  const X6Tile t = pick_tile_x6(p, MODE, Mrows_max, phases, P);
  if (t.kernel == X6Tile::Tap) {
    if (t.bn == 128) return launch_igemm_x6t<128, MODE, P>(p, Mrows_max, st);
    if (t.bn == 64) return launch_igemm_x6t<64, MODE, P>(p, Mrows_max, st);
    return launch_igemm_x6t<32, MODE, P>(p, Mrows_max, st);
  }
  if constexpr (P == 2) {
    if (t.kernel == X6Tile::Persistent) return launch_igemm_x6p<MODE>(p, Mrows_max, st);
  }
  if constexpr (MODE == 1 && P != 2) {
    if (p.bnb_x) return launch_igemm_x6_tile<1, P, true>(p, t, Mrows_max, phases, st);
  }
  return launch_igemm_x6_tile<MODE, P, false>(p, t, Mrows_max, phases, st);
}

int launch_igemm_x6(const IgemmParams& p, int mode, int Mrows_max, int phases, int pieces, hipStream_t st) {
  if (pieces == 2) {
    if (mode == 0) XAS_REQUIRE(p.a_amax, "conv: an f16x3 forward launch needs the maximum of its input tensor (xas_conv_shape.grad_amax)");
    else XAS_REQUIRE(p.a_amax && !p.bnb_x, "conv: an f16x3 data gradient needs the maximum of its gradient operand (xas_conv_shape.grad_amax)");
  }
  return with_pieces(pieces, [&](auto pc) {
    constexpr int P = decltype(pc)::value;
    return mode == 0 ? launch_igemm_x6_p<0, P>(p, Mrows_max, phases, st) : launch_igemm_x6_p<1, P>(p, Mrows_max, phases, st);
  });
}

template <int BMN>
struct XStride { static constexpr int value = BMN * 2 + (BMN == 128 ? 64 : (BMN == 64 ? 64 : 0)); };

template <int BM, int BN, int P>
__global__ __launch_bounds__(256, (P == 2 ? XAS_WX6_WAVES2 : 2)) void wgrad_x6_kernel(WgradParams p) {
  using C = TileCfg<BM, BN>;
  constexpr int SA = XStride<BM>::value, SB = XStride<BN>::value;
  constexpr int ASZ = P * XH * SA, BSZ = P * XH * SB, HBUF = ASZ + BSZ;
  constexpr int AQ = BM / 4, AROWS = 256 / AQ;
  constexpr int AK = WBK / AROWS;
  constexpr bool AHALF = AK == 1;
  constexpr int APH = AHALF ? 1 : AK / 2;
  constexpr int ASET = AHALF ? 1 : 2 * APH;
  constexpr int BPQ = BN / 64;
  static_assert(AK >= 1 && BPQ >= 1, "tile too small for the staging scheme");
  extern __shared__ __align__(16) float lds[];
  unsigned char* S = reinterpret_cast<unsigned char*>(lds);
  const int tid = threadIdx.x, lane = tid & 63, wave = tid >> 6;
  const int wm = wave / C::WAVES_N, wn = wave % C::WAVES_N;
  const int nkt = p.ntiles / p.nct;
  const int xcd = blockIdx.x & 7, qb = blockIdx.x >> 3;
  int split, tile;
  if (p.tune & XAS_TUNE_WGRAD_SPLIT_XCD) {
    split = xcd + 8 * (qb / p.ntiles);
    const int t = qb - (qb / p.ntiles) * p.ntiles;
    tile = (t / nkt) + (t - (t / nkt) * nkt) * p.nct;
  } else {
    const int grp = xcd + 8 * (qb / nkt);
    const int kt = qb - (qb / nkt) * nkt;
    split = grp / p.nct;
    tile = (grp - split * p.nct) + kt * p.nct;
  }
  if (split >= p.nsplits) return;
  const int co0 = (tile % p.nct) * BM, nn0 = (tile / p.nct) * BN;
  const int mbeg = split * p.m_per_split, mend = min(p.M, mbeg + p.m_per_split);
  const int HWo = p.Ho * p.Wo;
  const F16WgradScales<P> f16(p);

  const int aq = tid % AQ, apix = tid / AQ;
  const __amdgpu_buffer_rsrc_t rsrcA =
      __builtin_amdgcn_make_buffer_rsrc(const_cast<float*>(p.dy), 0, (int)((long)mend * p.Cout * 4), 0x00020000);
  const unsigned voffA = (co0 + aq * 4 < p.Cout) ? (unsigned)(apix * p.Cout + co0 + aq * 4) * 4u : kOOB;
  const unsigned passA = (unsigned)(AROWS * p.Cout) * 4u;
  const unsigned dstA = (unsigned)((apix & (XH - 1)) * SA + aq * 8);
  const int ahalf = __builtin_amdgcn_readfirstlane(apix >> 4);

  const int bq = tid & 15, bpix = tid >> 4;
  const long biasB = ((long)p.pad * p.Wi + p.pad) * p.Cin;
  const __amdgpu_buffer_rsrc_t rsrcB = __builtin_amdgcn_make_buffer_rsrc(
      const_cast<float*>(p.x) - biasB, 0, (int)((biasB + (long)p.N * p.Hi * p.Wi * p.Cin) * 4), 0x00020000);
  int tr[BPQ], ts[BPQ];
  unsigned offq[BPQ];
  bool colok[BPQ];
#pragma unroll
  for (int q = 0; q < BPQ; ++q) {
    const int nn = nn0 + (bq + 16 * q) * 4;
    colok[q] = nn < p.KK;
    const int nc = colok[q] ? nn : 0;
// ... 33 lines not shown
        rb[h * BPQ + q] = buf_load16(rsrcB, ok ? pix + offq[q] : kOOB, 0u);
      }
    }
  };
  auto store_half = [&](int buf, int h, const float4 (&ra)[ASET], const float4 (&rb)[2 * BPQ]) {
    unsigned char* sb = S + buf * HBUF;
#pragma unroll
    for (int j = 0; j < APH; ++j) {
      if (AHALF && ahalf != h) continue;
      const Pieces<P> pcs = split_pieces<P>(ra[AHALF ? 0 : h * APH + j], f16.sd);
#pragma unroll
      for (int pc = 0; pc < P; ++pc) *reinterpret_cast<uint2*>(sb + pc * XH * SA + AROWS * j * SA + dstA) = pcs.q[pc];
    }
#pragma unroll
    for (int q4 = 0; q4 < BPQ; ++q4) {
      const Pieces<P> pcs = split_pieces<P>(rb[h * BPQ + q4], f16.sx);
#pragma unroll
      for (int pc = 0; pc < P; ++pc) *reinterpret_cast<uint2*>(sb + pc * XH * SB + q4 * 128 + dstB) = pcs.q[pc];
    }
  };
  const int l16 = lane & 15, qd = l16 >> 2, pp = l16 & 3, g1 = (lane >> 4) & 1, hh = lane >> 5;
  const unsigned fragA = (unsigned)((8 * hh + qd) * SA + (wm * C::WM + 16 * g1 + 4 * pp) * 2);
  const unsigned fragB = (unsigned)(ASZ + (8 * hh + qd) * SB + (wn * C::WN + 16 * g1 + 4 * pp) * 2);
  auto compute = [&](int buf) {
    const unsigned char* sb = S + buf * HBUF;
    uint4 fa[P][C::MI], fb[P][C::NI];
#pragma unroll
    for (int pc = P - 1; pc >= 0; --pc) {
#pragma unroll
      for (int mi = 0; mi < C::MI; ++mi) fa[pc][mi] = tr_frag(sb, fragA + pc * XH * SA + mi * 64, SA);
#pragma unroll
      for (int ni = 0; ni < C::NI; ++ni) fb[pc][ni] = tr_frag(sb, fragB + pc * XH * SB + ni * 64, SB);
    }
    mfma_products<P, false>(acc, fa, fb);
  };
  const int nsteps = (mend > mbeg) ? (mend - mbeg + WBK - 1) / WBK : 0;
  const int last = nsteps - 1;
  auto mk_of = [&](int st) { return mbeg + (st < last ? st : last) * WBK; };
  if (nsteps > 0) {
    load_k(mk_of(0), ra_0, rb_0);
    load_k(mk_of(1), ra_1, rb_1);
    store_half(0, 0, ra_0, rb_0);
    int st = 0;
    for (; st + 1 < nsteps; st += 2) {
      __syncthreads();
      compute(0);
      store_half(1, 1, ra_0, rb_0);
      __syncthreads();
      load_k(mk_of(st + 2), ra_0, rb_0);
      compute(1);
      store_half(0, 0, ra_1, rb_1);
      __syncthreads();
      compute(0);
      store_half(1, 1, ra_1, rb_1);
      __syncthreads();
      load_k(mk_of(st + 3), ra_1, rb_1);
      compute(1);
      store_half(0, 0, ra_0, rb_0);
    }
    if (st < nsteps) {
      __syncthreads();
      compute(0);
      store_half(1, 1, ra_0, rb_0);
      __syncthreads();
      compute(1);
    }
  }
  float* slab = p.out + (size_t)split * p.Cout * p.KK;
  const int col_l = lane & 31, rsub = 4 * (lane >> 5);
#pragma unroll
  for (int mi = 0; mi < C::MI; ++mi)
#pragma unroll
    for (int reg = 0; reg < 16; ++reg) {
      const int co = co0 + wm * C::WM + mi * 32 + (reg & 3) + 8 * (reg >> 2) + rsub;
      if (co >= p.Cout) continue;
#pragma unroll
      for (int ni = 0; ni < C::NI; ++ni) {
        const int nn = nn0 + wn * C::WN + ni * 32 + col_l;
        if (nn < p.KK) slab[(size_t)co * p.KK + nn] = P == 2 ? acc[mi][ni][reg] * f16.desc : acc[mi][ni][reg];
      }
    }
}

template <int BM, int P>
__global__ __launch_bounds__(256, 2) void wgrad_x6t_kernel(WgradParams p) {
  constexpr int NCB = BM / 32, NTG = 4 / NCB;
  constexpr int NTW = (9 + NTG - 1) / NTG;
  constexpr int SA = XStride<BM>::value;
  constexpr int DYB = P * XH * SA;
  constexpr int XPB = 64;
  constexpr int DQ = BM / 4;
  constexpr int DJ = (XH * DQ + 255) / 256;
  extern __shared__ __align__(16) float lds[];
  unsigned char* S = reinterpret_cast<unsigned char*>(lds);
  const int tid = threadIdx.x, lane = tid & 63;
  const int wave = __builtin_amdgcn_readfirstlane(tid >> 6);
  const int cb = wave % NCB, tg = wave / NCB;
  const int H = p.Ho, W = p.Wo;
  const PatchGeom g(p.t2d_tw, H, W);
  const int xplane = g.npix * XPB;
  unsigned char* SX = S + 2 * DYB;
  const int nci = p.Cin / 32;
  const int tiles = p.nct * nci;
  const int split = blockIdx.x / tiles, tile = blockIdx.x - split * tiles;
  const int co0 = (tile / nci) * BM, c0 = (tile - (tile / nci) * nci) * 32;
  const int np_total = p.M >> 7;
  const int pbeg = split * p.pps, pend = min(np_total, pbeg + p.pps);
  if (pbeg >= pend) return;
  const F16WgradScales<P> f16(p);

  const __amdgpu_buffer_rsrc_t rsrcX = __builtin_amdgcn_make_buffer_rsrc(const_cast<float*>(p.x), 0, (int)((long)p.N * H * W * p.Cin * 4), 0x00020000);
  const __amdgpu_buffer_rsrc_t rsrcD = __builtin_amdgcn_make_buffer_rsrc(const_cast<float*>(p.dy), 0, (int)((long)p.M * p.Cout * 4), 0x00020000);
  int hpy[XT_NJ], hpx[XT_NJ], hpt[XT_NJ];
#pragma unroll
  for (int j = 0; j < XT_NJ; ++j) {
    const int item = tid + 256 * j, pix = item >> 3;
    hpt[j] = -1; hpy[j] = 0; hpx[j] = 0;
    if (pix < g.npix) g.halo_pixel(pix, hpt[j], hpy[j], hpx[j]);
  }
  float4 rx[XT_NJ];
  auto load_x = [&](int patch) {
    int img0, y0, x0;
    g.origin(patch, img0, y0, x0);
#pragma unroll
    for (int j = 0; j < XT_NJ; ++j) {
      const int gy = y0 + hpy[j], gx = x0 + hpx[j], img = img0 + hpt[j];
      const bool ok = hpt[j] >= 0 && g.inside(img, gy, gx, p.N);
      const unsigned off = ok ? (unsigned)((g.pixel(img, gy, gx) * p.Cin + c0 + ((tid + 256 * j) & 7) * 4) * 4) : kOOB;
      rx[j] = buf_load16(rsrcX, off, 0u);
    }
  };
  auto stage_x = [&]() {
#pragma unroll
    for (int j = 0; j < XT_NJ; ++j) {
      const int item = tid + 256 * j, pix = item >> 3, q = item & 7;
      if (pix < g.npix) {
        const Pieces<P> pcs = split_pieces<P>(rx[j], f16.sx);
        unsigned char* d = SX + pix * XPB + q * 8;
#pragma unroll
        for (int pc = 0; pc < P; ++pc) *reinterpret_cast<uint2*>(d + pc * xplane) = pcs.q[pc];
      }
    }
  };
  float4 rd[DJ];
  auto slice_row0 = [&](int patch, int ks) {
    int img0, y0, x0;
    g.origin(patch, img0, y0, x0);
    if (g.tw == 16) return (img0 * H + y0 + ks) * W + x0;
    return ((img0 + (ks >> 2)) * H + y0 + 2 * (ks & 3)) * W + x0;
  };
  auto load_dy = [&](int patch, int ks) {
    const unsigned soff = (unsigned)slice_row0(patch, ks) * (unsigned)p.Cout * 4u;
#pragma unroll
    for (int j = 0; j < DJ; ++j) {
      const int item = tid + 256 * j, apix = item / DQ, aq = item - apix * DQ;
      const bool ok = item < XH * DQ && co0 + aq * 4 < p.Cout;
      rd[j] = buf_load16(rsrcD, ok ? (unsigned)(apix * p.Cout + co0 + aq * 4) * 4u : kOOB, soff);
    }
  };
  auto store_dy = [&](int buf) {
    unsigned char* sb = S + buf * DYB;
#pragma unroll
    for (int j = 0; j < DJ; ++j) {
      const int item = tid + 256 * j, apix = item / DQ, aq = item - apix * DQ;
      if (item < XH * DQ) {
        const Pieces<P> pcs = split_pieces<P>(rd[j], f16.sd);
#pragma unroll
        for (int pc = 0; pc < P; ++pc) *reinterpret_cast<uint2*>(sb + pc * XH * SA + apix * SA + aq * 8) = pcs.q[pc];
      }
    }
  };
  const int l16 = lane & 15, qd = l16 >> 2, pp = l16 & 3, g1 = (lane >> 4) & 1, hh = lane >> 5;
  const unsigned fragA = (unsigned)((8 * hh + qd) * SA + (cb * 32 + 16 * g1 + 4 * pp) * 2);
  const int rs = g.tw == 16 ? 8 : g.hw;
  const unsigned fragX = (unsigned)((hh * rs + qd) * XPB + (16 * g1 + 4 * pp) * 2);
  f32x16 acc[NTW][1][1];
  zero_acc(acc);
  auto compute = [&](int buf, int ks) {
    const unsigned char* sb = S + buf * DYB;
    uint4 fa[P][1];
#pragma unroll
    for (int pc = P - 1; pc >= 0; --pc) fa[pc][0] = tr_frag(sb, fragA + pc * XH * SA, SA);
    const int wbase = g.tw == 16 ? (ks + 1) * g.hw + 1 : (ks >> 2) * g.npix_img + (2 * (ks & 3) + 1) * g.hw + 1;
#pragma unroll
    for (int ti = 0; ti < NTW; ++ti) {
      const int t = tg + ti * NTG;
      if (t < 9) {
        const int dy = t / 3 - 1, dx = t - (t / 3) * 3 - 1;
        const unsigned xo = (unsigned)((wbase + dy * g.hw + dx) * XPB) + fragX;
        uint4 fb[P][1];
#pragma unroll
        for (int pc = P - 1; pc >= 0; --pc) fb[pc][0] = tr_frag(SX, xo + pc * xplane, XPB);
        mfma_products<P, false>(acc[ti], fa, fb);
      }
    }
  };
  load_x(pbeg);
  load_dy(pbeg, 0);
  int buf = 0;
  for (int patch = pbeg; patch < pend; ++patch) {
    __syncthreads();
    stage_x();
    if (patch + 1 < pend) load_x(patch + 1);
    for (int ks = 0; ks < 8; ++ks) {
      store_dy(buf);
      if (ks < 7) load_dy(patch, ks + 1);
      else if (patch + 1 < pend) load_dy(patch + 1, 0);
      __syncthreads();
      compute(buf, ks);
      buf ^= 1;
    }
  }
  float* slab = p.out + (size_t)split * p.Cout * p.KK;
  const int col_l = lane & 31, rsub = 4 * (lane >> 5);
#pragma unroll
  for (int ti = 0; ti < NTW; ++ti) {
    const int t = tg + ti * NTG;
    if (t < 9) {
#pragma unroll
      for (int reg = 0; reg < 16; ++reg) {
        const int co = co0 + cb * 32 + (reg & 3) + 8 * (reg >> 2) + rsub;
        if (co < p.Cout) slab[(size_t)co * p.KK + t * p.Cin + c0 + col_l] = P == 2 ? acc[ti][0][0][reg] * f16.desc : acc[ti][0][0][reg];
      }
    }
  }
}

bool wgrad_x6t_plan(const xas_conv_shape* s, int* bm, int* splits, int* pps) {
  if (!tap_tile_ok(s->R, s->S, s->stride, s->pad, s->Hi, s->Wi, s->Ho, s->Wo, s->Cin, s->N)) return false;
  if (s->Cout != 64 && s->Cout != 32) return false;
  *bm = s->Cout;
  const long np = (long)s->N * s->Hi * s->Wi / 128;
  const long tiles = s->Cin / 32;
#ifndef XAS_WX6T_BLOCKS
#define XAS_WX6T_BLOCKS 1536
#endif
  long sp = cdiv(XAS_WX6T_BLOCKS, tiles);
  if (sp > np / 2) sp = np / 2;
  if (sp < 1) sp = 1;
  *pps = (int)cdiv(np, sp);
  *splits = (int)cdiv(np, *pps);
  return true;
}

template <int BM, int P>
static int launch_wgrad_x6t_t(const WgradParams& p, int splits, int pps, hipStream_t st) {
  constexpr size_t lds = (size_t)2 * P * XH * XStride<BM>::value + (size_t)P * 200 * 64;
  static bool attr_set_dev[kMaxDevices] = {};
  bool& attr_set = attr_set_dev[current_device()];
  if (!attr_set && lds > 64 * 1024) {
    (void)hipFuncSetAttribute(reinterpret_cast<const void*>(&wgrad_x6t_kernel<BM, P>), hipFuncAttributeMaxDynamicSharedMemorySize, (int)lds);
    attr_set = true;
  }
  WgradParams q = p;
  q.nct = p.Cout / BM;
  q.nsplits = splits; q.pps = pps;
  q.t2d_tw = p.Wo % 16 == 0 ? 16 : 8;
  dim3 grid((unsigned)(splits * q.nct * (p.Cin / 32)));
  hipLaunchKernelGGL((wgrad_x6t_kernel<BM, P>), grid, dim3(256), lds, st, q);
  XAS_LAUNCH_CHECK();
  return 0;
}

int launch_wgrad_x6t(const WgradParams& p, int bm, int splits, int pps, int pieces, hipStream_t st) {
  if (pieces == 2)
    XAS_REQUIRE(p.a_amax && p.b_amax, "conv_wgrad: the f16x3 weight gradient needs the maxima of both tensor operands (xas_conv_shape.grad_amax, x_amax)");
  return with_pieces(pieces, [&](auto pc) {
    constexpr int P = decltype(pc)::value;
    return bm == 64 ? launch_wgrad_x6t_t<64, P>(p, splits, pps, st) : launch_wgrad_x6t_t<32, P>(p, splits, pps, st);
  });
}

template <int BM, int BN, int P>
static int launch_wgrad_x6_t(const WgradParams& p, int splits, hipStream_t st) {
  constexpr size_t lds = (size_t)2 * P * XH * (XStride<BM>::value + XStride<BN>::value);
  WgradParams q = p;
  q.nct = (int)cdiv(p.Cout, BM);
  q.ntiles = q.nct * (int)cdiv(p.KK, BN);
  q.nsplits = splits;
  q.tune = (splits % 8 == 0) ? XAS_TUNE_WGRAD_SPLIT_XCD : 0;
  dim3 grid(q.tune ? (unsigned)(splits * q.ntiles) : (unsigned)(8 * cdiv((long)splits * q.nct, 8) * (q.ntiles / q.nct)));
  hipLaunchKernelGGL((wgrad_x6_kernel<BM, BN, P>), grid, dim3(256), lds, st, q);
  XAS_LAUNCH_CHECK();
  return 0;
}

int launch_wgrad_x6(const WgradParams& p, int bm, int bn, int splits, int pieces, hipStream_t st) {
  if (pieces == 2)
    XAS_REQUIRE(p.a_amax && p.b_amax, "conv_wgrad: the f16x3 weight gradient needs the maxima of both tensor operands (xas_conv_shape.grad_amax, x_amax)");
  return with_pieces(pieces, [&](auto pc) {
    constexpr int P = decltype(pc)::value;
    if (bm == 32) return launch_wgrad_x6_t<32, 128, P>(p, splits, st);
    if (bm == 128) return bn == 128 ? launch_wgrad_x6_t<128, 128, P>(p, splits, st) : launch_wgrad_x6_t<128, 64, P>(p, splits, st);
    return bn == 128 ? launch_wgrad_x6_t<64, 128, P>(p, splits, st) : launch_wgrad_x6_t<64, 64, P>(p, splits, st);
  });
}

}

using namespace xas;

__global__ __launch_bounds__(256) void prepare_weights_kernel(const long* __restrict__ d, int n) {
  int lo = 0, hi = n - 1;
  while (lo < hi) {
    const int mid = (lo + hi + 1) >> 1;
    if (d[mid * 12 + 10] <= (long)blockIdx.x) lo = mid; else hi = mid - 1;
  }
  const long* e = d + lo * 12;
  const float* src = reinterpret_cast<const float*>(e[0]);
  unsigned short* dst = reinterpret_cast<unsigned short*>(e[1]);
  const int Cout = (int)e[2], Cin = (int)e[3], R = (int)e[4], S = (int)e[5], transposed = (int)e[6], P = (int)e[7];
  const int rows = (int)e[8], K = (int)e[9];
  const int nhc = K / 16;
  const long total = (long)((rows + 31) / 32) * nhc * 64;
  const long id = ((long)blockIdx.x - e[10]) * 256 + threadIdx.x;
  if (id >= total) return;
  const int lane = (int)(id & 63);
  const long blk = id >> 6;
  const int hc = (int)(blk % nhc), rb = (int)(blk / nhc);
  const int row = rb * 32 + (lane & 31), k0 = hc * 16 + (lane >> 5) * 8;
  float v[8];
#pragma unroll
  for (int j = 0; j < 8; ++j) {
    v[j] = 0.f;
    if (row < rows) {
      const int k = k0 + j;
      int co, ci, tap;
      if (!transposed) { ci = k % Cin; tap = k / Cin; co = row; }
      else { co = k % Cout; tap = k / Cout; ci = row; }
      const int q = tap % S, r = tap / S;
      v[j] = src[(((long)co * Cin + ci) * R + r) * S + q];
    }
  }
  float4 r0 = make_float4(v[0], v[1], v[2], v[3]), r1 = make_float4(v[4], v[5], v[6], v[7]);
  unsigned short* o = dst + (blk * P) * 512 + lane * 8;
  switch (P) {
    case 3: split_store_weight<3>(r0, r1, o); break;
    case 2: split_store_weight<2>(r0, r1, o); break;
    default: split_store_weight<1>(r0, r1, o); break;
  }
}

extern "C" int xas_prepare_weights(const void* descs, int n, long blocks, void* stream) {
  XAS_REQUIRE(descs && n > 0 && blocks > 0 && blocks < 0x7fffffffl, "prepare_weights: bad arguments");
  hipLaunchKernelGGL(prepare_weights_kernel, dim3((unsigned)blocks), dim3(256), 0, as_stream(stream), reinterpret_cast<const long*>(descs), n);
  XAS_LAUNCH_CHECK();
  return 0;
}

// ... 45 lines not shown
```

x-as-supervision_amd/modules/physique_network.py:

```python
import torch.nn as nn

from xas_amd import layers as L
from xas_amd import ops_nn as F
from xas_amd.ops_nn import ACT_LEAKY


class PhysiqueMaskGenerator(nn.Module):
    def __init__(self, num_features, num_parts=1):
        super().__init__()
        self.num_features = num_features
        self.num_parts = num_parts
        self.encoder, self.decoder = self.define_network(num_features)

    @staticmethod
    def _unit(cin, cout, stride=1, up=False):
        mods = [L.Upsample2x()] if up else []
        mods += [L.Conv2d(cin, cout, 3, stride=stride, padding=1, bias=True),
                 L.BatchNorm2d(cout, act=ACT_LEAKY, sync=True), nn.Identity()]
        return nn.Sequential(*mods)

    def define_network(self, f):
        enc = [self._unit(self.num_parts, f[0])]
        for i in range(1, len(f)):
            enc += [self._unit(f[i - 1], f[i - 1]), self._unit(f[i - 1], f[i], stride=2)]
        dec = []
        for i in range(len(f) - 1, 0, -1):
            dec += [self._unit(f[i], f[i]), self._unit(f[i], f[i - 1], up=True)]
        dec.append(L.Conv2d(f[0], 1, 3, stride=1, padding=1, bias=True))
        return nn.Sequential(*enc), nn.Sequential(*dec)

    def forward(self, input):
        return F.sigmoid(self.decoder(self.encoder(input)))

    def forward_groups(self, input, groups):
        with F.bn_groups(groups):
            return F.sigmoid(self.decoder(self.encoder(input)))
```

x-as-supervision_amd/xas_amd/_lib.py:

```python
import ctypes
import os

import torch

_HERE = os.path.dirname(os.path.abspath(__file__))
LIB_PATH = os.environ.get('XAS_HIP_LIB') or os.path.join(_HERE, 'libxas_hip.so')
_lib = None
ABI_VERSION = 3

_T = {'p': ctypes.c_void_p, 'i': ctypes.c_int, 'l': ctypes.c_long, 'f': ctypes.c_float, 'u': ctypes.c_uint,
      'd': ctypes.c_double, 'z': ctypes.c_size_t}


class ConvShape(ctypes.Structure):
    _fields_ = [(n, ctypes.c_int) for n in ('N', 'Hi', 'Wi', 'Cin', 'Cout', 'R', 'S', 'stride', 'pad', 'Ho', 'Wo', 'mode')] + [
        ('grad_amax', ctypes.c_void_p),
        ('x_amax', ctypes.c_void_p)]


PREC_F32, PREC_BF16, PREC_BF16X6, PREC_F16X3 = 0, 1, 2, 3
PREC_NAMES = {'f32': PREC_F32, 'bf16': PREC_BF16, 'bf16x6': PREC_BF16X6, 'f16x3': PREC_F16X3}

GUARD_FLOATS = 8
GUARD_NORM, GUARD_SCALE, GUARD_SKIP, GUARD_T, GUARD_SKIPPED, GUARD_STEP_SIZE, GUARD_INV_SQRT_BC2, GUARD_NONFINITE = range(8)

TUNE_WGRAD_SPLIT_XCD = 1
TUNE_PLAIN_KLOOP, TUNE_GLOBAL_LOAD, TUNE_WGRAD_GLOBAL_LOAD = 32, 64, 128
TUNE_WGRAD_ALT_ORDER, TUNE_WGRAD_PLAIN_KLOOP = 8192, 524288
TUNE_SLAB_SHIFT, TUNE_SLAB_MASK = 15, 3
TUNE_SLAB_512, TUNE_SLAB_128, TUNE_SLAB_64 = 32768, 65536, 98304
TUNE_COL_REDUCE_LEAN = 262144
TUNE_GENERAL_KERNELS = 1 << 22
TUNE_NO_WIDE_TILES, TUNE_NO_STEM_WGRAD, TUNE_STEM_FWD_F32 = 1 << 23, 1 << 24, 1 << 25
TUNE_NO_X6P, TUNE_X6P_ANY_K = 1 << 26, 1 << 27

PLAN_FIELDS = ('route', 'kernel', 'bm', 'bn', 'pipelined', 'phases', 'pieces', 'patch_width', 'tpb', 'images')
PLAN_ROUTES = (None, 'stem_f16', 'stem_f32', 'thin_vec_to_scalar', 'thin_scalar_to_vec', 'direct', 'mfma')
PLAN_KERNELS = (None, 'igemm_buf', 'igemm', 'igemm_x6', 'igemm_x6t', 'igemm_x6p')


def conv_igemm_plan(shp, pass_, has_bias=False):
    out = (ctypes.c_int * len(PLAN_FIELDS))()
    rc = fn('xas_conv_igemm_plan')(shp, pass_, int(has_bias), ctypes.cast(out, ctypes.c_void_p))
    if rc != 0:
        raise RuntimeError('xas_conv_igemm_plan failed (%d): %s' % (rc, load().xas_last_error().decode()))
    plan = dict(zip(PLAN_FIELDS, out))
    plan['route'], plan['kernel'] = PLAN_ROUTES[plan['route']], PLAN_KERNELS[plan['kernel']]
    return plan


SIGNATURES = {
    'xas_abi_version': ('', 'i'),
    'xas_set_tuning': ('i', 'i'),
    'xas_set_precision': ('i', 'i'),
    'xas_get_precision': ('', 'i'),
    'xas_conv_weight_planes': ('si', 'i'),
    'xas_conv_kernel_class': ('si', 'i'),
    'xas_f16_weight_overflow': ('i', 'i'),
    'xas_f16_weight_overflow_peek': ('pp', 'i'),
    'xas_split_weight_bytes': ('lli', 'z'),
    'xas_split_weight': ('ppllip', 'i'),
    'xas_prepare_weights': ('pilp', 'i'),
    'xas_head_workspace_floats': ('iii', 'z'),
    'xas_head_softargmax_fwd': ('piiiiipppippp', 'i'),
    'xas_head_softargmax_bwd': ('ppppiiiiippp', 'i'),
    'xas_head_softargmax_bwd_amax': ('ppppiiiiipppp', 'i'),
    'xas_patch_to_world_fwd': ('ppppppiiiffipp', 'i'),
    'xas_patch_to_world_bwd': ('pppppppiiiffipp', 'i'),
    'xas_world_to_patch_fwd': ('ppfipppppiiiffipp', 'i'),
    'xas_world_to_patch_bwd': ('pppfipppppiiiffippp', 'i'),
    'xas_lines_nblk': ('i', 'i'),
    'xas_draw_lines_max_fwd': ('plliippiufipp', 'i'),
    'xas_draw_lines_max_bwd': ('plliippiufipppp', 'i'),
    'xas_conv_fwd': ('ppppsp', 'i'),
    'xas_conv_fwd_head_chunks': ('sii', 'i'),
    'xas_conv_fwd_head': ('ppppsiipp', 'i'),
    'xas_head_softargmax_from_partials': ('piiiiiipppipp', 'i'),
    'xas_head_softargmax_flip_from_partials': ('piiiiiippppip', 'i'),
    'xas_head_softargmax_fwd_flip': ('piiiiippppipp', 'i'),
    'xas_head_spread_workspace_floats': ('iii', 'z'),
    'xas_head_spread': ('piiippp', 'i'),
    'xas_conv_fwd_bnstats_workspace_floats': ('si', 'z'),
    'xas_conv_fwd_bnstats': ('pppsippplppppfp', 'i'),
    'xas_conv_dgrad_bn_bwd_workspace_floats': ('si', 'z'),
    'xas_conv_dgrad_bn_bwd': ('ppspppppfidppppppp', 'i'),
    'xas_conv_dgrad': ('pppsp', 'i'),
    'xas_conv_dgrad_acc': ('pppsp', 'i'),
    'xas_conv_dgrad_acc_masked': ('pppsppp', 'i'),
    'xas_conv_igemm_plan': ('siip', 'i'),
    'xas_conv_wgrad_workspace_floats': ('s', 'z'),
    'xas_conv_wgrad': ('ppppsp', 'i'),
    'xas_conv_wgrad_oihw': ('ppppsp', 'i'),
    'xas_conv_wgrad_acc': ('ppppsp', 'i'),
    'xas_pack_weight': ('ppiiiiip', 'i'),
    'xas_unpack_weight': ('ppiiiiip', 'i'),
    'xas_bn_workspace_floats': ('lii', 'z'),
    'xas_bn_stats': ('pliipplppppflp', 'i'),
    'xas_bn_stats_from_partials': ('pliilppplppppfp', 'i'),
    'xas_bn_bwd_sums_from_partials': ('pliippppp', 'i'),
    'xas_bn_sync_merge': ('piiilppppfp', 'i'),
    'xas_col_sum': ('plippp', 'i'),
    'xas_col_sum_acc': ('plippp', 'i'),
    'xas_bn_apply': ('ppppppfiliippp', 'i'),
    'xas_bn_apply_amax': ('ppppppfiliipppp', 'i'),
    'xas_abs_max': ('plpp', 'i'),
    'xas_bn_update_running': ('ppppfliip', 'i'),
    'xas_bn_bwd_reduce': ('pppppppfiliipppppp', 'i'),
    'xas_bn_bwd_apply': ('ppppppppfiliidpppp', 'i'),
    'xas_bn_bwd_apply_amax': ('ppppppppfiliidppppp', 'i'),
    'xas_bn_apply_dual_amax': ('pppppf' 'pppppf' 'lii' 'pppp', 'i'),
    'xas_bn_bwd_reduce_dual': ('ppppppf' 'ppf' 'lii' 'ppp' 'pppp' 'p', 'i'),
    'xas_bn_bwd_apply_dual_amax': ('pppp' 'ppppf' 'ppppf' 'liidd' 'pppp' 'p', 'i'),
    'xas_maxpool3x3s2_fwd': ('piiiippp', 'i'),
    'xas_maxpool3x3s2_bwd': ('ppiiiipp', 'i'),
    'xas_upsample2x_fwd': ('piiiipp', 'i'),
    'xas_upsample2x_bwd': ('piiiipp', 'i'),
    'xas_sigmoid_fwd': ('plpp', 'i'),
    'xas_sigmoid_bwd': ('pplpp', 'i'),
    'xas_nchw_to_nhwc': ('piiiipp', 'i'),
    'xas_nhwc_to_nchw': ('piiiipp', 'i'),
    'xas_nchw_to_nhwc_mirror_pair': ('piiiipp', 'i'),
    'xas_warp_affine_u8': ('ppppiiipp', 'i'),
    'xas_mask_blur_threshold': ('piipp', 'i'),
    'xas_patch_finish': ('pppppiiippp', 'i'),
    'xas_geodesic_workspace_bytes': ('ii', 'z'),
    'xas_geodesic_weight': ('pppiipppp', 'i'),
    'xas_geodesic_weight_multi': ('ppiipiipppp', 'i'),
    'xas_loss_nblk': ('l', 'i'),
    'xas_mask_loss_fwd': ('pppliPpp'.replace('P', 'p'), 'i'),
    'xas_mask_loss_bwd': ('pppliPppp'.replace('P', 'p'), 'i'),
    'xas_pose_loss_fwd': ('ppiiiifffpp', 'i'),
    'xas_pose_loss_bwd': ('ppiiiifffppppp', 'i'),
    'xas_lsgan_fwd': ('piifppp', 'i'),
    'xas_lsgan_bwd': ('piifpppp', 'i'),
    'xas_graph_aggregate': ('ppiiipp', 'i'),
    'xas_gln_workspace_floats': ('lii', 'z'),
    'xas_gln_fwd': ('ppppliifpppp', 'i'),
    'xas_gln_bwd': ('pppppliifppppp', 'i'),
    'xas_smpl_lbs_fwd': ('ppppppppiiipppp', 'i'),
    'xas_smpl_lbs_bwd_workspace_floats': ('ii', 'z'),
# ... 87 lines not shown
```

x-as-supervision_amd/xas_amd/layers.py:

```python
import math

import torch
import torch.distributed as dist
import torch.nn as nn

from . import ops_nn as F


def _kaiming_fan_out_(w):
    fan_out = w.shape[0] * w[0][0].numel()
    with torch.no_grad():
        w.normal_(0.0, math.sqrt(2.0 / fan_out))


class Conv2d(nn.Module):
    def __init__(self, cin, cout, k, stride=1, padding=0, bias=True, init='default'):
        super().__init__()
        self.stride, self.padding = stride, padding
        self.weight = nn.Parameter(torch.empty(cout, cin, k, k))
        self.bias = nn.Parameter(torch.zeros(cout)) if bias else None
        if init == 'kaiming_fan_out':
            _kaiming_fan_out_(self.weight)
        else:
            nn.init.kaiming_uniform_(self.weight, a=math.sqrt(5))
# ... 1 lines not shown
                bound = 1 / math.sqrt(cin * k * k)
                nn.init.uniform_(self.bias, -bound, bound)
        self._cache = F._PackCache()
        self.head_kd = None

    def forward(self, x):
        return F.conv2d(x, self.weight, self.bias, self.stride, self.padding, self._cache, self.head_kd)


class ConvTranspose2d(nn.Module):

    def __init__(self, cin, cout, k, stride, padding):
        super().__init__()
        self.stride, self.padding = stride, padding
        self.weight = nn.Parameter(torch.empty(cin, cout, k, k))
        _kaiming_fan_out_(self.weight)
        self._cache = F._PackCache()

    def forward(self, x):
        return F.conv_transpose2d(x, self.weight, self.stride, self.padding, self._cache)


class Linear(nn.Module):
    def __init__(self, cin, cout, bias=True):
        super().__init__()
        self.weight = nn.Parameter(torch.empty(cout, cin))
        self.bias = nn.Parameter(torch.zeros(cout)) if bias else None
        nn.init.kaiming_uniform_(self.weight, a=math.sqrt(5))
        if bias:
            bound = 1 / math.sqrt(cin)
            nn.init.uniform_(self.bias, -bound, bound)
        self._cache = F._PackCache()

    def forward(self, x):
        return F.linear(x, self.weight, self.bias, self._cache)


class BatchNorm2d(nn.Module):

    def __init__(self, c, act=F.ACT_NONE, sync=False, eps=1e-5, momentum=0.1):
        super().__init__()
        self.act, self.sync, self.eps, self.momentum = act, sync, eps, momentum
        self.weight = nn.Parameter(torch.ones(c))
        self.bias = nn.Parameter(torch.zeros(c))
        self.register_buffer('running_mean', torch.zeros(c))
        self.register_buffer('running_var', torch.ones(c))
        self.register_buffer('num_batches_tracked', torch.tensor(0, dtype=torch.long))
        self._nbt_shared = False

    def sync_group(self):
        if self.sync and self.training:
            from .dp import dp_active
            if dp_active():
                return dist.group.WORLD
        return None

    def count_batch(self):
        if self.training and not self._nbt_shared:
            from . import streams
            n = F.current_groups()
            if streams.forked():
                with torch.cuda.stream(streams.book_stream()):
                    self.num_batches_tracked += n
            else:
                self.num_batches_tracked += n

    def forward(self, x, residual=None):
        group = self.sync_group()
        self.count_batch()
        return F.batch_norm(x, self.weight, self.bias, self.running_mean, self.running_var, residual, self.training,
                            self.momentum, self.eps, self.act, group)


class MaxPool3x3s2(nn.Module):
    def forward(self, x):
        return F.maxpool3x3s2(x)


class Upsample2x(nn.Module):
    def forward(self, x):
        return F.upsample2x(x)


class SharedBatchCounters:

    def __init__(self, net):
        self.net = net
        self.arena = None

    def _bind(self):
        mods = [m for m in self.net.modules() if isinstance(m, BatchNorm2d)]
        dev = mods[0].num_batches_tracked.device
        arena = torch.stack([m.num_batches_tracked.reshape(()) for m in mods]).to(dev)
        for i, m in enumerate(mods):
            m._buffers['num_batches_tracked'] = arena[i]
            m._nbt_shared = True
        self.arena, self.mods = arena, mods

    def bump(self):
        ok = self.arena is not None and all(
            m._buffers['num_batches_tracked'].data_ptr() == self.arena.data_ptr() + 8 * i for i, m in enumerate(self.mods))
        if not ok:
            self._bind()
        from . import streams
        n = F.current_groups()
        if streams.forked():
            with torch.cuda.stream(streams.book_stream()):
                self.arena += n
        else:
            self.arena += n
```

x-as-supervision_amd/xas_amd/ops_nn.py:

```python
import os

import torch
import torch.distributed as dist

from . import _lib
from . import streams
from ._lib import ConvShape, call, ptr, query

CL = torch.channels_last
_weights_epoch = [0]

_groups = [1]

_prefix = [0, 0]


class bn_groups:
    def __init__(self, groups, prefix_groups=0, images_per_group=0):
        self.groups = int(groups)
        self.prefix = [int(prefix_groups) * int(images_per_group), int(prefix_groups)]
        if self.prefix[1] and not (0 < self.prefix[1] < self.groups and images_per_group > 0):
            raise RuntimeError('bn_groups: the no-grad prefix must be a proper, non-empty subset of the groups')

    def __enter__(self):
# ... 1039 lines not shown


class _BatchNorm(torch.autograd.Function):
    @staticmethod
    def forward(ctx, x, gamma, beta, running_mean, running_var, residual, training, momentum, eps, act, group):
        y, saved, cfg = _bn_forward(x, gamma, beta, running_mean, running_var, residual, training, momentum, eps, act, group)
        ctx.save_for_backward(*saved, gamma, beta)
        ctx.cfg = cfg
        if ctx.needs_input_grad[1] and ctx.needs_input_grad[2]:
            note_use(gamma)
            note_use(beta)
        return y

    @staticmethod
    def backward(ctx, dy):
        *saved, gamma, beta = ctx.saved_tensors
        dx, dgamma, dbeta, dres = _bn_backward(tuple(saved), ctx.cfg, gamma, beta, dy,
                                               ctx.needs_input_grad[1] and ctx.needs_input_grad[2])
        return dx, dgamma, dbeta, None, None, dres, None, None, None, None, None


def batch_norm(x, gamma, beta, running_mean, running_var, residual=None, training=True, momentum=0.1, eps=1e-5,
               act=ACT_NONE, group=None):
    return _BatchNorm.apply(x, gamma, beta, running_mean, running_var, residual, training, momentum, eps, act, group)


class _MaxPool(torch.autograd.Function):
    @staticmethod
    def forward(ctx, x):
        x = to_cl(x)
        n, c, h, w = x.shape
        ho, wo = (h - 1) // 2 + 1, (w - 1) // 2 + 1
        xf = _full(x)
        nf = xf.shape[0]
        yf = empty_cl(nf, c, ho, wo, x)
        idxf = torch.empty(nf * ho * wo * c, device=x.device, dtype=torch.int8)
        call('xas_maxpool3x3s2_fwd', ptr(xf), nf, h, w, c, ptr(yf), ptr(idxf))
        y, idx = _tail(yf), _tail(idxf, per_image=ho * wo * c)
        pass_amax(y, x)
        ctx.save_for_backward(idx)
        ctx.shape = (n, c, h, w)
        return y

    @staticmethod
    def backward(ctx, dy):
        (idx,) = ctx.saved_tensors
        n, c, h, w = ctx.shape
        dy = to_cl(dy)
        dx = empty_cl(n, c, h, w, dy)
        call('xas_maxpool3x3s2_bwd', ptr(dy), ptr(idx), n, h, w, c, ptr(dx))
        return dx


def maxpool3x3s2(x):
    return _MaxPool.apply(x)


class _Upsample2x(torch.autograd.Function):
    @staticmethod
    def forward(ctx, x):
        if _prefix[0]:
            raise RuntimeError('prefix pass: up-sampling is not on the detector path')
        x = to_cl(x)
        n, c, h, w = x.shape
        y = empty_cl(n, c, 2 * h, 2 * w, x)
        call('xas_upsample2x_fwd', ptr(x), n, h, w, c, ptr(y))
        pass_amax(y, x)
        ctx.shape = (n, c, h, w)
        return y

    @staticmethod
    def backward(ctx, dy):
        n, c, h, w = ctx.shape
        dy = to_cl(dy)
        dx = empty_cl(n, c, h, w, dy)
        call('xas_upsample2x_bwd', ptr(dy), n, h, w, c, ptr(dx))
        return dx


def upsample2x(x):
    return _Upsample2x.apply(x)


class _Sigmoid(torch.autograd.Function):
    @staticmethod
    def forward(ctx, x):
        x = x.contiguous() if x.dim() != 4 else to_cl(x)
        y = torch.empty_like(x)
        call('xas_sigmoid_fwd', ptr(x), x.numel(), ptr(y))
        ctx.save_for_backward(y)
        return y

    @staticmethod
    def backward(ctx, dy):
        (y,) = ctx.saved_tensors
        dy = dy.contiguous() if dy.dim() != 4 else to_cl(dy)
        dx = torch.empty_like(y)
        call('xas_sigmoid_bwd', ptr(y), ptr(dy), y.numel(), ptr(dx))
        return dx


def sigmoid(x):
    return _Sigmoid.apply(x)


BATCH_PREP = os.environ.get('XAS_BATCH_PREP', '1') != '0'


def _conv_entries(module):
    out = []
    for m in module.modules():
        cache = getattr(m, '_cache', None)
        w = getattr(m, 'weight', None)
        if isinstance(cache, _PackCache) and w is not None and w.dim() == 4 and w.is_cuda:
            a, b, r, s = w.shape
            stride, pad = int(getattr(m, 'stride', 1)), int(getattr(m, 'padding', 0))
            if type(m).__name__ == 'ConvTranspose2d':
                hs = 8
                hb = (hs - 1) * stride - 2 * pad + r
                shp = _shape(1, hb, hb, b, a, r, s, stride, pad, hs, hs)
            else:
                hi = 16
                ho = (hi + 2 * pad - r) // stride + 1
                shp = _shape(1, hi, hi, b, a, r, s, stride, pad, ho, ho)
            out.append((m, cache, w, shp))
        elif isinstance(cache, _PackCache) and w is not None and w.dim() == 2 and w.is_cuda and LINEAR_MFMA and w.is_contiguous() \
                and w.shape[1] % 32 == 0 and w.shape[0] >= 16 and w.shape[0] % 4 == 0:
            co, ci = w.shape
            w4 = w.detach().view(co, ci, 1, 1)
            w4._xas_epoch = getattr(w, '_xas_epoch', _weights_epoch)
            shp = _shape(1, 8, 32, ci, co, 1, 1, 1, 0, 8, 32)
            shp._linear = True
            out.append((m, cache, w4, shp))
    return out


def prepack(module):
    entries = _conv_entries(module)
    if not entries:
        return
    prec = query('xas_get_precision')
    if not BATCH_PREP:
        for _, cache, w, shp in entries:
            if getattr(shp, '_linear', False):
                cache.get(w, 0, shp)
                cache.get(w, 1, shp)
                continue
            f16 = (prec == _lib.PREC_F16X3 and GRAD_F16 and shp.mode == 0 and query('xas_conv_weight_planes', shp, 1) == 3)
            if not (f16 and query('xas_conv_weight_planes', shp, 0) == 3):
                cache.get(w, 0, shp)
            cache.get(w, 1, shp)
            if f16:
                cache.get(w, 0, shp, planes=2)
                cache.get(w, 1, shp, planes=2)
        return
    key = (prec, tuple(w.data_ptr() for _, _, w, _ in entries))
    tab = getattr(module, '_xas_prep', None)
    if tab is None or tab['key'] != key:
        rows_of, views, desc, blk, off = [], [], [], 0, 0
        sizes = []
        for idx, (_, cache, w, shp) in enumerate(entries):
            lin = getattr(shp, '_linear', False)
            f16 = prec == _lib.PREC_F16X3 and GRAD_F16 and shp.mode == 0 and not lin
            for t, extra in ((0, False), (1, False), (0, True), (1, True)):
                planes = query('xas_conv_weight_planes', shp, t)
                if lin and extra:
# ... 39 lines not shown
```

x-as-supervision_amd/xas_amd/prof.py:

```python
import torch

from . import _lib

CONV_ENTRIES = ('xas_conv_fwd', 'xas_conv_fwd_head', 'xas_conv_fwd_bnstats', 'xas_conv_dgrad', 'xas_conv_dgrad_acc', 'xas_conv_dgrad_acc_masked', 'xas_conv_wgrad',
                'xas_conv_wgrad_oihw', 'xas_conv_wgrad_acc')


BN_ENTRIES = ('xas_bn_stats', 'xas_bn_apply', 'xas_bn_apply_amax', 'xas_bn_bwd_reduce', 'xas_bn_bwd_apply', 'xas_bn_bwd_apply_amax',
              'xas_bn_apply_dual_amax', 'xas_bn_bwd_reduce_dual', 'xas_bn_bwd_apply_dual_amax')


def bn_bytes(name, a):
    if name == 'xas_bn_stats':
        return 4.0 * a[1] * a[2]
    if name in ('xas_bn_apply', 'xas_bn_apply_amax'):
        t = 4.0 * a[8] * a[9]
        return t * (2 + (1 if a[5] else 0)) + (t / 16 if a[12] else 0.0)
    if name == 'xas_bn_bwd_reduce':
        t = 4.0 * a[9] * a[10]
        return t * (1 + (1 if a[0] else 0) + (1 if a[1] else 0)) + (t / 16 if a[16] else 0.0)
    if name == 'xas_bn_apply_dual_amax':
        t = 4.0 * a[12] * a[13]
        return t * 3 + t / 16
    if name == 'xas_bn_bwd_reduce_dual':
        t = 4.0 * a[10] * a[11]
        return t * 3 + t / 16
    if name == 'xas_bn_bwd_apply_dual_amax':
        t = 4.0 * a[14] * a[15]
        return t * 5 + t / 16
    t = 4.0 * a[10] * a[11]
    return t * (2 + (1 if a[0] else 0) + (1 if a[1] else 0) + (1 if a[15] else 0)) + (t / 16 if a[16] else 0.0)


def conv_flops(shape):
    return 2.0 * shape.N * shape.Ho * shape.Wo * shape.Cout * shape.R * shape.S * shape.Cin


def conv_bytes(shape):
    return 4.0 * (shape.N * shape.Hi * shape.Wi * shape.Cin + shape.Cout * shape.R * shape.S * shape.Cin
                  + shape.N * shape.Ho * shape.Wo * shape.Cout)


class KernelTimer:
    def __init__(self, names=CONV_ENTRIES):
        self.names = set(names)
        self.records = []
        self.bytes_total = 0.0

    def __enter__(self):
        _lib.profiler = self
        return self

    def __exit__(self, *exc):
        _lib.profiler = None

    def timed_call(self, name, args):
        shape = next((a for a in args if isinstance(a, _lib.ConvShape)), None)
        a, b = torch.cuda.Event(enable_timing=True), torch.cuda.Event(enable_timing=True)
        a.record()
        rc = _lib.fn(name)(*args, _lib.stream())
        b.record()
        if rc != 0:
            raise RuntimeError('%s failed (%d): %s' % (name, rc, _lib.load().xas_last_error().decode()))
        mfma = 0
        if shape is not None:
            kind = 0 if name in ('xas_conv_fwd', 'xas_conv_fwd_head', 'xas_conv_fwd_bnstats') else (
                1 if name in ('xas_conv_dgrad', 'xas_conv_dgrad_acc', 'xas_conv_dgrad_acc_masked', 'xas_conv_dgrad_bn_bwd') else 2)
            mfma = _lib.query('xas_conv_kernel_class', shape, kind)
        sig = None
        if shape is not None:
            sig = (shape.N, shape.Hi, shape.Wi, shape.Cin, shape.Cout, shape.R, shape.stride)
        work = conv_flops(shape) if shape is not None else 0.0
        if name == 'xas_head_softargmax_fwd':
            B, K, D = args[1], args[2], args[3]
            work, sig = 4.0 * B * K * D * D * D, (B, K, D)
        elif name == 'xas_head_softargmax_from_partials':
            B, K, D, nch = args[1], args[2], args[3], args[4]
            work, sig = 4.0 * B * nch * K * (3 + D), (B, K, D)
        elif name in BN_ENTRIES:
            work, sig = bn_bytes(name, args), None
        elif name in ('xas_head_softargmax_bwd', 'xas_head_softargmax_bwd_amax'):
            B, K, D = args[4], args[5], args[6]
            work, sig = 8.0 * B * K * D * D * D, (B, K, D)
        self.records.append((name, a, b, work, mfma, sig))
        self.bytes_total += conv_bytes(shape) if (shape is not None and mfma) else 0.0

    CLASS = {0: ':direct', 1: ':f32', 2: ':bf16', 3: ':bf16x6', 4: ':f16x3'}

    def summary(self):
        out = {}
        for name, a, b, fl, mfma, _sig in self.records:
            key = name + (self.CLASS[mfma] if name.startswith('xas_conv') else '')
            d = out.setdefault(key, {'launches': 0, 'ms': 0.0, 'flops': 0.0})
            d['launches'] += 1
            d['ms'] += a.elapsed_time(b)
            d['flops'] += fl
        return out

    def by_shape(self):
        agg = {}
        for name, a, b, fl, mfma, sig in self.records:
            d = agg.setdefault((name, sig), [0, 0.0, 0.0])
            d[0] += 1
            d[1] += a.elapsed_time(b)
            d[2] += fl
        rows = [(k[0], k[1], v[0], v[1], (v[2] / (v[1] * 1e-3) / 1e12) if v[1] > 0 else 0.0) for k, v in agg.items()]
        return sorted(rows, key=lambda r: -r[3])
```

Measured before the change: 2107 images/s.

## Fuse bilinear x2 upsample into forward and weight-gradient conv operand loads

Adds an up-sampled-operand mode to the tap igemm forward kernel and the split-tap weight-gradient kernel. These kernels load the half-resolution source patch into LDS and interpolate it on the fly, so the upsampled activation is never written to or read from global memory. Decoder up-conv blocks switch to a fused autograd function when the kernels accept the shape. The backward data gradient still goes through a separate upsample backward. The trade-off is extra LDS use, an added barrier and interpolation arithmetic in the staging loop, which may reduce occupancy.

```diff
diff --git a/include/xas_hip.h b/include/xas_hip.h
--- a/include/xas_hip.h
+++ b/include/xas_hip.h
@@ -106,6 +106,9 @@
   const float* grad_amax;
   const float* x_amax;
 } xas_conv_shape;
+
+enum { XAS_X_UP2 = 0x200 };
+int xas_conv_up2_fused(const xas_conv_shape* s, int pass);
 
 int xas_conv_weight_planes(const xas_conv_shape* s, int pass);
 int xas_conv_kernel_class(const xas_conv_shape* s, int pass);
diff --git a/x-as-supervision_amd/csrc/bn.hip b/x-as-supervision_amd/csrc/bn.hip
--- a/x-as-supervision_amd/csrc/bn.hip
+++ b/x-as-supervision_amd/csrc/bn.hip
@@ -793,12 +793,7 @@
   const float4 b = *reinterpret_cast<const float4*>(base + ((size_t)h0 * W + w1) * C);
   const float4 cc = *reinterpret_cast<const float4*>(base + ((size_t)h1 * W + w0) * C);
   const float4 d = *reinterpret_cast<const float4*>(base + ((size_t)h1 * W + w1) * C);
-  const float h0l = 1.f - lh, w0l = 1.f - lw;
-  float4 o;
-  o.x = h0l * (w0l * a.x + lw * b.x) + lh * (w0l * cc.x + lw * d.x);
-  o.y = h0l * (w0l * a.y + lw * b.y) + lh * (w0l * cc.y + lw * d.y);
-  o.z = h0l * (w0l * a.z + lw * b.z) + lh * (w0l * cc.z + lw * d.z);
-  o.w = h0l * (w0l * a.w + lw * b.w) + lh * (w0l * cc.w + lw * d.w);
+  const float4 o = up2_interp4(a, b, cc, d, lh, lw);
   stream_store(reinterpret_cast<float4*>(y + ((size_t)row * Wo + wo) * C + c), o);
 }
 
diff --git a/x-as-supervision_amd/csrc/common.h b/x-as-supervision_amd/csrc/common.h
--- a/x-as-supervision_amd/csrc/common.h
+++ b/x-as-supervision_amd/csrc/common.h
@@ -56,6 +56,25 @@
   return __fmaf_rn(__fsub_rn(x, m), rs_g, b);
 }
 
+__device__ __forceinline__ float up2_interp_xz(float a, float b, float c, float d, float lh, float lw) {
+  const float h0l = 1.f - lh, w0l = 1.f - lw;
+  const float top = __fmaf_rn(lw, b, __fmul_rn(w0l, a)), bot = __fmaf_rn(w0l, c, __fmul_rn(lw, d));
+  return __fmaf_rn(lh, bot, __fmul_rn(h0l, top));
+}
+__device__ __forceinline__ float up2_interp_yw(float a, float b, float c, float d, float lh, float lw) {
+  const float h0l = 1.f - lh, w0l = 1.f - lw;
+  const float top = __fmaf_rn(w0l, a, __fmul_rn(lw, b)), bot = __fmaf_rn(w0l, c, __fmul_rn(lw, d));
+  return __fmaf_rn(h0l, top, __fmul_rn(lh, bot));
+}
+__device__ __forceinline__ float4 up2_interp4(float4 a, float4 b, float4 c, float4 d, float lh, float lw) {
+  return make_float4(up2_interp_xz(a.x, b.x, c.x, d.x, lh, lw), up2_interp_yw(a.y, b.y, c.y, d.y, lh, lw),
+                     up2_interp_xz(a.z, b.z, c.z, d.z, lh, lw), up2_interp_yw(a.w, b.w, c.w, d.w, lh, lw));
+}
+__device__ __forceinline__ void up2_coord(int o, int n, int& i0, int& i1, float& l) {
+  const float s = fmaxf(0.f, (o + 0.5f) * 0.5f - 0.5f);
+  i0 = (int)s; i1 = min(i0 + 1, n - 1); l = s - i0;
+}
+
 __device__ __forceinline__ void stream_store(float4* p, float4 v) {
 #ifndef XAS_NO_NT_STORES
   typedef float f32x4_nt_t __attribute__((ext_vector_type(4)));
diff --git a/x-as-supervision_amd/csrc/conv.hip b/x-as-supervision_amd/csrc/conv.hip
--- a/x-as-supervision_amd/csrc/conv.hip
+++ b/x-as-supervision_amd/csrc/conv.hip
@@ -1542,6 +1542,27 @@
   return {s->N * Hp * Wp, s->stride * s->stride};
 }
 
+static bool fwd_up2_launch_fused(const xas_conv_shape* s) {
+  if (((s->Hi | s->Wi) & 1) || fwd_route(s, true) != FwdRoute::Mfma || precision_of(s) == XAS_PREC_F32) return false;
+  const int pieces = planes_of(precision_of(s), 0, has_amax_for(s, 0));
+  const IgemmGrid g = fwd_grid(s);
+  return igemm_up2_takes(pick_tile_x6(fwd_problem(s), 0, g.Mrows_max, g.phases, pieces), pieces);
+}
+static bool wgrad_up2_launch_fused(const xas_conv_shape* s, bool x_aligned) {
+  if (((s->Hi | s->Wi) & 1) || (s->mode & XAS_GRAD_IS_X)) return false;
+  return wgrad_route(s, x_aligned).kernel == WgradKernel::SplitTap && wgrad_up2_takes(planes_of(precision_of(s), 2, has_amax_for(s, 2)));
+}
+extern "C" int xas_conv_up2_fused(const xas_conv_shape* s, int pass) {
+  if (!s || (pass != 0 && pass != 2) || s->N < 1 || s->Hi < 1 || s->Wi < 1 || s->Cin < 1 || s->Cout < 1) return 0;
+  const long xi = (long)s->Hi * s->Wi * s->Cin, yi = (long)s->Ho * s->Wo * s->Cout;
+  bool all = true;
+  (void)for_image_ranges(s, pass == 0 ? fwd_images_per_launch(s) : images_per_launch(s->N, xi, yi), [&](int, const xas_conv_shape* part) {
+    all = all && (pass == 0 ? fwd_up2_launch_fused(part) : wgrad_up2_launch_fused(part, true));
+    return 0;
+  });
+  return all ? 1 : 0;
+}
+
 static int fwd_stats_tile_rows(const xas_conv_shape* s, int groups) {
   if (!s || groups < 1) return 0;
   if (fwd_route(s, false) != FwdRoute::Mfma || s->Cout % 4 != 0) return 0;
@@ -1571,7 +1592,8 @@
                          void* stream, float* stat_partial, const float* stat_pivot, float* head_partial = nullptr) {
   if (check_shape(s, "conv_fwd") || check_fwd_dims(s, "conv_fwd")) return 1;
   XAS_REQUIRE(x && w_packed && y, "conv_fwd: null buffer");
-  const long xi = (long)s->Hi * s->Wi * s->Cin, yi = (long)s->Ho * s->Wo * s->Cout;
+  const bool up2 = (s->mode & XAS_X_UP2) != 0;
+  const long xi = (long)s->Hi * s->Wi * s->Cin / (up2 ? 4 : 1), yi = (long)s->Ho * s->Wo * s->Cout;
   const int per = fwd_images_per_launch(s);
   if (per < s->N) {
     XAS_REQUIRE(!stat_partial, "conv_fwd: the statistics epilogue needs a single launch");
@@ -1581,6 +1603,7 @@
     });
   }
   hipStream_t st = as_stream(stream);
+  if (up2) XAS_REQUIRE(fwd_up2_launch_fused(s), "conv_fwd: no kernel takes this shape / precision with a x2 up-sampled operand (ask xas_conv_up2_fused)");
   const FwdRoute route = fwd_route(s, bias != nullptr);
   switch (route) {
     case FwdRoute::StemF16:
@@ -1610,6 +1633,7 @@
   p.src = x; p.wgt = w_packed; p.bias = bias; p.out = y;
   p.stat_partial = stat_partial; p.stat_pivot = stat_pivot;
   p.head_partial = head_partial;
+  if (up2) { p.up2 = 1; p.src_elems /= 4; }
   const IgemmGrid g = fwd_grid(s);
   return dispatch_igemm<0>(p, precision_of(s), g.Mrows_max, g.phases, st);
 }
@@ -1934,13 +1958,15 @@
   if (check_shape(s, "conv_wgrad")) return 1;
   XAS_REQUIRE(x && dy && dw_packed && workspace, "conv_wgrad: null buffer");
   XAS_REQUIRE(s->Cout % 4 == 0 || s->Cout == 1, "conv_wgrad: Cout=%d must be a multiple of 4 (or 1)", s->Cout);
+  const bool up2 = (s->mode & XAS_X_UP2) != 0;
   const long xi = (long)s->Hi * s->Wi * s->Cin, yi = (long)s->Ho * s->Wo * s->Cout;
   const int per = images_per_launch(s->N, xi, yi);
   if (per < s->N && (oihw || accumulate))
     return for_image_ranges(s, per, [&](int n0, const xas_conv_shape* part) {
-      return conv_wgrad_impl(x + (size_t)n0 * xi, dy + (size_t)n0 * yi, dw_packed, workspace, part, stream, oihw, accumulate || n0 > 0);
+      return conv_wgrad_impl(x + (size_t)n0 * (xi / (up2 ? 4 : 1)), dy + (size_t)n0 * yi, dw_packed, workspace, part, stream, oihw, accumulate || n0 > 0);
     });
   hipStream_t st = as_stream(stream);
+  if (up2) XAS_REQUIRE(wgrad_up2_launch_fused(s, ((uintptr_t)x & 15) == 0), "conv_wgrad: no kernel takes this shape / precision with a x2 up-sampled operand (ask xas_conv_up2_fused)");
   const WgradRoute r = wgrad_route(s, ((uintptr_t)x & 15) == 0);
   switch (r.kernel) {
     case WgradKernel::Thin: {
@@ -2004,6 +2030,7 @@
   p.KK = s->R * s->S * s->Cin; p.M = s->N * s->Ho * s->Wo; p.m_per_split = r.m_per_split;
   p.div_hw.init((unsigned)(s->Ho * s->Wo)); p.div_w.init((unsigned)s->Wo);
   p.div_cin.init((unsigned)s->Cin); p.div_s.init((unsigned)s->S);
+  p.up2 = up2 ? 1 : 0;
   const int pieces = planes_of(precision_of(s), 2, has_amax_for(s, 2));
   int rc;
   switch (r.kernel) {
diff --git a/x-as-supervision_amd/csrc/conv_shared.h b/x-as-supervision_amd/csrc/conv_shared.h
--- a/x-as-supervision_amd/csrc/conv_shared.h
+++ b/x-as-supervision_amd/csrc/conv_shared.h
@@ -52,6 +52,7 @@
   float* bnb_partial;
   const float* a_amax;
   float* head_partial;
+  int up2;
 };
 
 constexpr int kMaxDevices = 16;
@@ -453,6 +454,7 @@
   int t2d_tw, pps;
   const float* a_amax; const float* b_amax;
   FastDiv div_hw, div_w, div_cin, div_s;
+  int up2;
 };
 
 constexpr int WBK = 32;
@@ -482,6 +484,8 @@
   enum Kernel { General, Tap, Persistent } kernel;
 };
 X6Tile pick_tile_x6(const IgemmParams& p, int mode, int Mrows_max, int phases, int pieces);
+bool igemm_up2_takes(const X6Tile& t, int pieces);
+bool wgrad_up2_takes(int pieces);
 int x6p_tiles_per_block(const IgemmParams& p, int Mrows_max);
 int launch_wgrad_x6(const WgradParams& p, int bm, int bn, int splits, int pieces, hipStream_t st);
 bool wgrad_x6t_plan(const xas_conv_shape* s, int* bm, int* splits, int* pps);
diff --git a/x-as-supervision_amd/csrc/conv_x6.hip b/x-as-supervision_amd/csrc/conv_x6.hip
--- a/x-as-supervision_amd/csrc/conv_x6.hip
+++ b/x-as-supervision_amd/csrc/conv_x6.hip
@@ -135,6 +135,45 @@
   }
   __device__ __forceinline__ long pixel(int img, int gy, int gx) const { return ((long)img * H + gy) * W + gx; }
 };
+
+constexpr int XU_PIXB = 128;
+constexpr int XU_NJ = 3;
+constexpr int XU_RAW_MAX = 72 * XU_PIXB;
+struct Up2Patch {
+  int Hh, Wh, sw, npix_img, npix, sy0, sx0;
+  __device__ __forceinline__ Up2Patch(const PatchGeom& g, int y0, int x0) {
+    Hh = g.H >> 1; Wh = g.W >> 1;
+    sw = (g.tw >> 1) + 2; npix_img = 6 * sw; npix = g.tn_cnt * npix_img;
+    sy0 = (y0 >> 1) - 1; sx0 = (x0 >> 1) - 1;
+  }
+  __device__ __forceinline__ unsigned source_offset(int item, int img0, int N, int C, int c0) const {
+    const int pix = item >> 3, q = item & 7;
+    if (pix >= npix) return kOOB;
+    const int tn = pix / npix_img, pr = pix - tn * npix_img, ry = pr / sw;
+    const int gy = sy0 + ry, gx = sx0 + (pr - ry * sw), img = img0 + tn;
+    if ((unsigned)gy >= (unsigned)Hh || (unsigned)gx >= (unsigned)Wh || img >= N) return kOOB;
+    return (unsigned)(((((long)img * Hh + gy) * Wh + gx) * C + c0 + q * 4) * 4);
+  }
+  __device__ __forceinline__ unsigned code(int tn, int gy, int gx, int q) const {
+    int h0, h1, w0, w1;
+    float lh, lw;
+    up2_coord(gy, Hh, h0, h1, lh);
+    up2_coord(gx, Wh, w0, w1, lw);
+    const unsigned off = (unsigned)(((tn * 6 + (h0 - sy0)) * sw + (w0 - sx0)) * XU_PIXB + q * 16);
+    return off | (unsigned)(h1 != h0) << 16 | (unsigned)(w1 != w0) << 17 | 1u << 18 | (unsigned)(int)(lh * 4.f) << 19 | (unsigned)(int)(lw * 4.f) << 21;
+  }
+  __device__ __forceinline__ float4 value(const unsigned char* raw, unsigned c) const {
+    if (!(c & (1u << 18))) return make_float4(0.f, 0.f, 0.f, 0.f);
+    const unsigned char* r = raw + (c & 0xffffu);
+    const int dh = (c >> 16 & 1u) ? sw * XU_PIXB : 0, dw = (c >> 17 & 1u) ? XU_PIXB : 0;
+    const float lh = (float)(c >> 19 & 3u) * 0.25f, lw = (float)(c >> 21 & 3u) * 0.25f;
+    return up2_interp4(*reinterpret_cast<const float4*>(r), *reinterpret_cast<const float4*>(r + dw),
+                       *reinterpret_cast<const float4*>(r + dh), *reinterpret_cast<const float4*>(r + dh + dw), lh, lw);
+  }
+};
+bool igemm_up2_takes(const X6Tile& t, int pieces) {
+  return t.kernel == X6Tile::Tap && (t.bn == 64 || t.bn == 32) && (pieces == 2 || pieces == 3);
+}
 
 __device__ unsigned g_f16_weight_overflow = 0u;
 __device__ __forceinline__ void f16_weight_check(float4 a, float4 b) {
@@ -451,8 +490,9 @@
 #ifndef XAS_X6T_WAVES
 #define XAS_X6T_WAVES 2
 #endif
-template <int BN, int MODE, int P>
+template <int BN, int MODE, int P, bool UP2 = false>
 __global__ __launch_bounds__(256, XAS_X6T_WAVES) void igemm_x6t_kernel(IgemmParams p) {
+  static_assert(!UP2 || MODE == 0, "the up-sampled operand exists for the forward pass only");
   constexpr int BM = 128;
   using C = TileCfg<BM, BN>;
   extern __shared__ __align__(16) float lds[];
@@ -489,18 +529,49 @@
       if (g.inside(img, gy, gx, p.N)) voffA[j] = (unsigned)((g.pixel(img, gy, gx) * p.Cs + q * 4) * 4);
     }
   }
-  float4 ra[XT_NJ];
+  const Up2Patch u(g, y0, x0);
+  unsigned char* SU = S + P * XT_PLANE_MAX;
+  unsigned ucode[UP2 ? XT_NJ : 1], voffU[UP2 ? XU_NJ : 1];
+  float4 ru[UP2 ? XU_NJ : 1];
+  if constexpr (UP2) {
+#pragma unroll
+    for (int j = 0; j < XT_NJ; ++j) {
+      const int item = tid + 256 * j, pix = item >> 3, q = item & 7;
+      ucode[j] = 0u;
+      if (pix < g.npix) {
+        int tn, dy, dx;
+        g.halo_pixel(pix, tn, dy, dx);
+        const int gy = y0 + dy, gx = x0 + dx;
+        if (g.inside(img0 + tn, gy, gx, p.N)) ucode[j] = u.code(tn, gy, gx, q);
+      }
+    }
+#pragma unroll
+    for (int j = 0; j < XU_NJ; ++j) voffU[j] = u.source_offset(tid + 256 * j, img0, p.N, p.Cs, 0);
+  }
+  float4 ra[UP2 ? 1 : XT_NJ];
   auto load_chunk = [&](int chunk) {
     const unsigned soff = (unsigned)(chunk * BK) * 4u;
-#pragma unroll
-    for (int j = 0; j < XT_NJ; ++j) ra[j] = buf_load16(rsrcA, voffA[j], soff);
+    if constexpr (UP2) {
+#pragma unroll
+      for (int j = 0; j < XU_NJ; ++j) ru[j] = buf_load16(rsrcA, voffU[j], soff);
+    } else {
+#pragma unroll
+      for (int j = 0; j < XT_NJ; ++j) ra[j] = buf_load16(rsrcA, voffA[j], soff);
+    }
+  };
+  auto store_raw = [&]() {
+#pragma unroll
+    for (int j = 0; j < (UP2 ? XU_NJ : 0); ++j)
+      if (tid + 256 * j < u.npix * 8) *reinterpret_cast<float4*>(SU + (tid + 256 * j) * 16) = ru[j];
   };
   auto stage = [&]() {
 #pragma unroll
     for (int j = 0; j < XT_NJ; ++j) {
       const int item = tid + 256 * j, pix = item >> 3, q = item & 7;
       if (pix < g.npix) {
-        const Pieces<P> pcs = split_pieces<P>(ra[j], f16.sa);
+        float4 v;
+        if constexpr (UP2) v = u.value(SU, ucode[j]); else v = ra[j];
+        const Pieces<P> pcs = split_pieces<P>(v, f16.sa);
         unsigned char* d = S + pix * XT_PIXB + q * 8;
 #pragma unroll
         for (int pc = 0; pc < P; ++pc) *reinterpret_cast<uint2*>(d + pc * plane_b) = pcs.q[pc];
@@ -550,6 +621,7 @@
   load_chunk(0);
   load_b(gb_0, 0);
   load_b(gb_1, 1);
+  if constexpr (UP2) { store_raw(); __syncthreads(); }
   for (int chunk = 0; chunk < cchunks; ++chunk) {
     stage();
     __syncthreads();
@@ -565,6 +637,7 @@
       mfma_products<P, true>(acc, fa_1, gb_1);
       load_b(gb_1, 1);
     }
+    if constexpr (UP2) store_raw();
     __syncthreads();
   }
   scale_acc<P>(acc, f16.desc);
@@ -572,8 +645,8 @@
 }
 
 template <int BN>
-constexpr size_t igemm_x6t_lds(int P) {
-  size_t a = (size_t)P * XT_PLANE_MAX;
+constexpr size_t igemm_x6t_lds(int P, bool up2 = false) {
+  size_t a = (size_t)P * XT_PLANE_MAX + (up2 ? XU_RAW_MAX : 0);
   size_t b = ((size_t)128 * (BN / (BN == 128 ? 2 : 1) + 4) + 2 * 256) * sizeof(float);
   return a > b ? a : b;
 }
@@ -624,15 +697,16 @@
   return 0;
 }
 
-template <int BN, int MODE, int P>
+template <int BN, int MODE, int P, bool UP2 = false>
 static int launch_igemm_x6t(const IgemmParams& p, int Mrows_max, hipStream_t st) {
-  constexpr size_t lds = igemm_x6t_lds<BN>(P);
+  constexpr size_t lds = igemm_x6t_lds<BN>(P, UP2);
+  static_assert(lds <= 64 * 1024, "igemm_x6t_kernel: beyond the default dynamic LDS limit");
   IgemmParams q = p;
   q.t2d_tw = tap_patch_width(p.Wd);
   q.nMt = Mrows_max / 128; q.nNt = (int)cdiv(p.Cd, BN);
   q.xn = 1; q.nt_per_x = q.nNt; q.mt_per_xcd = (int)cdiv(q.nMt, 8);
   dim3 grid((unsigned)(8 * q.mt_per_xcd * q.nt_per_x), 1, 1);
-  hipLaunchKernelGGL((igemm_x6t_kernel<BN, MODE, P>), grid, dim3(256), lds, st, q);
+  hipLaunchKernelGGL((igemm_x6t_kernel<BN, MODE, P, UP2>), grid, dim3(256), lds, st, q);
   XAS_LAUNCH_CHECK();
   return 0;
 }
@@ -706,6 +780,13 @@
 template <int MODE, int P>
 static int launch_igemm_x6_p(const IgemmParams& p, int Mrows_max, int phases, hipStream_t st) {
   const X6Tile t = pick_tile_x6(p, MODE, Mrows_max, phases, P);
+  if (p.up2) {
+    if constexpr (MODE == 0 && P >= 2) {
+      if (igemm_up2_takes(t, P)) return t.bn == 64 ? launch_igemm_x6t<64, 0, P, true>(p, Mrows_max, st) : launch_igemm_x6t<32, 0, P, true>(p, Mrows_max, st);
+    }
+    set_error("conv: no kernel takes this shape with a x2 up-sampled operand (xas_conv_up2_fused tells)");
+    return 1;
+  }
   if (t.kernel == X6Tile::Tap) {
     if (t.bn == 128) return launch_igemm_x6t<128, MODE, P>(p, Mrows_max, st);
     if (t.bn == 64) return launch_igemm_x6t<64, MODE, P>(p, Mrows_max, st);
@@ -905,7 +986,7 @@
     }
 }
 
-template <int BM, int P>
+template <int BM, int P, bool UP2 = false>
 __global__ __launch_bounds__(256, 2) void wgrad_x6t_kernel(WgradParams p) {
   constexpr int NCB = BM / 32, NTG = 4 / NCB;
   constexpr int NTW = (9 + NTG - 1) / NTG;
@@ -932,7 +1013,7 @@
   if (pbeg >= pend) return;
   const F16WgradScales<P> f16(p);
 
-  const __amdgpu_buffer_rsrc_t rsrcX = __builtin_amdgcn_make_buffer_rsrc(const_cast<float*>(p.x), 0, (int)((long)p.N * H * W * p.Cin * 4), 0x00020000);
+  const __amdgpu_buffer_rsrc_t rsrcX = __builtin_amdgcn_make_buffer_rsrc(const_cast<float*>(p.x), 0, (int)((long)p.N * (UP2 ? H >> 1 : H) * (UP2 ? W >> 1 : W) * p.Cin * 4), 0x00020000);
   const __amdgpu_buffer_rsrc_t rsrcD = __builtin_amdgcn_make_buffer_rsrc(const_cast<float*>(p.dy), 0, (int)((long)p.M * p.Cout * 4), 0x00020000);
   int hpy[XT_NJ], hpx[XT_NJ], hpt[XT_NJ];
 #pragma unroll
@@ -941,24 +1022,46 @@
     hpt[j] = -1; hpy[j] = 0; hpx[j] = 0;
     if (pix < g.npix) g.halo_pixel(pix, hpt[j], hpy[j], hpx[j]);
   }
-  float4 rx[XT_NJ];
+  float4 rx[UP2 ? 1 : XT_NJ], ru[UP2 ? XU_NJ : 1];
+  unsigned char* SU = SX + P * 200 * XPB;
   auto load_x = [&](int patch) {
     int img0, y0, x0;
     g.origin(patch, img0, y0, x0);
-#pragma unroll
-    for (int j = 0; j < XT_NJ; ++j) {
-      const int gy = y0 + hpy[j], gx = x0 + hpx[j], img = img0 + hpt[j];
-      const bool ok = hpt[j] >= 0 && g.inside(img, gy, gx, p.N);
-      const unsigned off = ok ? (unsigned)((g.pixel(img, gy, gx) * p.Cin + c0 + ((tid + 256 * j) & 7) * 4) * 4) : kOOB;
-      rx[j] = buf_load16(rsrcX, off, 0u);
-    }
-  };
-  auto stage_x = [&]() {
+    if constexpr (UP2) {
+      const Up2Patch u(g, y0, x0);
+#pragma unroll
+      for (int j = 0; j < XU_NJ; ++j) ru[j] = buf_load16(rsrcX, u.source_offset(tid + 256 * j, img0, p.N, p.Cin, c0), 0u);
+    } else {
+#pragma unroll
+      for (int j = 0; j < XT_NJ; ++j) {
+        const int gy = y0 + hpy[j], gx = x0 + hpx[j], img = img0 + hpt[j];
+        const bool ok = hpt[j] >= 0 && g.inside(img, gy, gx, p.N);
+        const unsigned off = ok ? (unsigned)((g.pixel(img, gy, gx) * p.Cin + c0 + ((tid + 256 * j) & 7) * 4) * 4) : kOOB;
+        rx[j] = buf_load16(rsrcX, off, 0u);
+      }
+    }
+  };
+  auto store_raw = [&]() {
+#pragma unroll
+    for (int j = 0; j < (UP2 ? XU_NJ : 0); ++j)
+      if (tid + 256 * j < g.tn_cnt * 6 * ((g.tw >> 1) + 2) * 8) *reinterpret_cast<float4*>(SU + (tid + 256 * j) * 16) = ru[j];
+  };
+  auto stage_x = [&](int patch) {
+    int img0 = 0, y0 = 0, x0 = 0;
+    if constexpr (UP2) g.origin(patch, img0, y0, x0);
+    const Up2Patch u(g, y0, x0);
 #pragma unroll
     for (int j = 0; j < XT_NJ; ++j) {
       const int item = tid + 256 * j, pix = item >> 3, q = item & 7;
       if (pix < g.npix) {
-        const Pieces<P> pcs = split_pieces<P>(rx[j], f16.sx);
+        float4 v;
+        if constexpr (UP2) {
+          const int gy = y0 + hpy[j], gx = x0 + hpx[j];
+          v = u.value(SU, g.inside(img0 + hpt[j], gy, gx, p.N) ? u.code(hpt[j], gy, gx, q) : 0u);
+        } else {
+          v = rx[j];
+        }
+        const Pieces<P> pcs = split_pieces<P>(v, f16.sx);
         unsigned char* d = SX + pix * XPB + q * 8;
 #pragma unroll
         for (int pc = 0; pc < P; ++pc) *reinterpret_cast<uint2*>(d + pc * xplane) = pcs.q[pc];
@@ -1020,10 +1123,11 @@
   };
   load_x(pbeg);
   load_dy(pbeg, 0);
+  if constexpr (UP2) store_raw();
   int buf = 0;
   for (int patch = pbeg; patch < pend; ++patch) {
     __syncthreads();
-    stage_x();
+    stage_x(patch);
     if (patch + 1 < pend) load_x(patch + 1);
     for (int ks = 0; ks < 8; ++ks) {
       store_dy(buf);
@@ -1032,6 +1136,9 @@
       __syncthreads();
       compute(buf, ks);
       buf ^= 1;
+    }
+    if constexpr (UP2) {
+      if (patch + 1 < pend) store_raw();
     }
   }
   float* slab = p.out + (size_t)split * p.Cout * p.KK;
@@ -1066,13 +1173,13 @@
   return true;
 }
 
-template <int BM, int P>
+template <int BM, int P, bool UP2 = false>
 static int launch_wgrad_x6t_t(const WgradParams& p, int splits, int pps, hipStream_t st) {
-  constexpr size_t lds = (size_t)2 * P * XH * XStride<BM>::value + (size_t)P * 200 * 64;
+  constexpr size_t lds = (size_t)2 * P * XH * XStride<BM>::value + (size_t)P * 200 * 64 + (UP2 ? XU_RAW_MAX : 0);
   static bool attr_set_dev[kMaxDevices] = {};
   bool& attr_set = attr_set_dev[current_device()];
   if (!attr_set && lds > 64 * 1024) {
-    (void)hipFuncSetAttribute(reinterpret_cast<const void*>(&wgrad_x6t_kernel<BM, P>), hipFuncAttributeMaxDynamicSharedMemorySize, (int)lds);
+    (void)hipFuncSetAttribute(reinterpret_cast<const void*>(&wgrad_x6t_kernel<BM, P, UP2>), hipFuncAttributeMaxDynamicSharedMemorySize, (int)lds);
     attr_set = true;
   }
   WgradParams q = p;
@@ -1080,14 +1187,21 @@
   q.nsplits = splits; q.pps = pps;
   q.t2d_tw = p.Wo % 16 == 0 ? 16 : 8;
   dim3 grid((unsigned)(splits * q.nct * (p.Cin / 32)));
-  hipLaunchKernelGGL((wgrad_x6t_kernel<BM, P>), grid, dim3(256), lds, st, q);
+  hipLaunchKernelGGL((wgrad_x6t_kernel<BM, P, UP2>), grid, dim3(256), lds, st, q);
   XAS_LAUNCH_CHECK();
   return 0;
 }
+
+bool wgrad_up2_takes(int pieces) { return pieces == 2 || pieces == 3; }
 
 int launch_wgrad_x6t(const WgradParams& p, int bm, int splits, int pps, int pieces, hipStream_t st) {
   if (pieces == 2)
     XAS_REQUIRE(p.a_amax && p.b_amax, "conv_wgrad: the f16x3 weight gradient needs the maxima of both tensor operands (xas_conv_shape.grad_amax, x_amax)");
+  if (p.up2) {
+    XAS_REQUIRE(wgrad_up2_takes(pieces), "conv_wgrad: no kernel takes this precision with a x2 up-sampled operand (xas_conv_up2_fused tells)");
+    if (pieces == 2) return bm == 64 ? launch_wgrad_x6t_t<64, 2, true>(p, splits, pps, st) : launch_wgrad_x6t_t<32, 2, true>(p, splits, pps, st);
+    return bm == 64 ? launch_wgrad_x6t_t<64, 3, true>(p, splits, pps, st) : launch_wgrad_x6t_t<32, 3, true>(p, splits, pps, st);
+  }
   return with_pieces(pieces, [&](auto pc) {
     constexpr int P = decltype(pc)::value;
     return bm == 64 ? launch_wgrad_x6t_t<64, P>(p, splits, pps, st) : launch_wgrad_x6t_t<32, P>(p, splits, pps, st);
diff --git a/x-as-supervision_amd/modules/physique_network.py b/x-as-supervision_amd/modules/physique_network.py
--- a/x-as-supervision_amd/modules/physique_network.py
+++ b/x-as-supervision_amd/modules/physique_network.py
@@ -17,7 +17,7 @@
         mods = [L.Upsample2x()] if up else []
         mods += [L.Conv2d(cin, cout, 3, stride=stride, padding=1, bias=True),
                  L.BatchNorm2d(cout, act=ACT_LEAKY, sync=True), nn.Identity()]
-        return nn.Sequential(*mods)
+        return L.UpConvSequential(*mods) if up else nn.Sequential(*mods)
 
     def define_network(self, f):
         enc = [self._unit(self.num_parts, f[0])]
diff --git a/x-as-supervision_amd/xas_amd/_lib.py b/x-as-supervision_amd/xas_amd/_lib.py
--- a/x-as-supervision_amd/xas_amd/_lib.py
+++ b/x-as-supervision_amd/xas_amd/_lib.py
@@ -56,6 +56,7 @@
     'xas_get_precision': ('', 'i'),
     'xas_conv_weight_planes': ('si', 'i'),
     'xas_conv_kernel_class': ('si', 'i'),
+    'xas_conv_up2_fused': ('si', 'i'),
     'xas_f16_weight_overflow': ('i', 'i'),
     'xas_f16_weight_overflow_peek': ('pp', 'i'),
     'xas_split_weight_bytes': ('lli', 'z'),
diff --git a/x-as-supervision_amd/xas_amd/layers.py b/x-as-supervision_amd/xas_amd/layers.py
--- a/x-as-supervision_amd/xas_amd/layers.py
+++ b/x-as-supervision_amd/xas_amd/layers.py
@@ -107,6 +107,18 @@
         return F.upsample2x(x)
 
 
+class UpConvSequential(nn.Sequential):
+
+    def forward(self, x):
+        up, conv = self[0], self[1]
+        if not (isinstance(up, Upsample2x) and isinstance(conv, Conv2d) and conv.stride == 1 and conv.head_kd is None):
+            raise RuntimeError('UpConvSequential: expected Upsample2x followed by a stride-1 Conv2d')
+        x = F.upsample2x_conv2d(x, conv.weight, conv.bias, conv.padding, conv._cache)
+        for m in list(self)[2:]:
+            x = m(x)
+        return x
+
+
 class SharedBatchCounters:
 
     def __init__(self, net):
diff --git a/x-as-supervision_amd/xas_amd/ops_nn.py b/x-as-supervision_amd/xas_amd/ops_nn.py
--- a/x-as-supervision_amd/xas_amd/ops_nn.py
+++ b/x-as-supervision_amd/xas_amd/ops_nn.py
@@ -1145,6 +1145,81 @@
     return _Upsample2x.apply(x)
 
 
+UP_FUSE = os.environ.get('XAS_UP_FUSE', '1') == '1'
+X_UP2 = 0x200
+up_stats = {'fused': 0, 'separate': 0}
+
+
+def _x_up2(shp):
+    out = ConvShape(shp.N, shp.Hi, shp.Wi, shp.Cin, shp.Cout, shp.R, shp.S, shp.stride, shp.pad, shp.Ho, shp.Wo,
+                    shp.mode | X_UP2, shp.grad_amax, shp.x_amax)
+    if hasattr(shp, '_slots'):
+        out._slots = shp._slots
+    return out
+
+
+def _up_conv_shape(x, weight, pad):
+    n, ci, h, w = x.shape
+    co, ci2, r, s = weight.shape
+    if ci != ci2:
+        raise RuntimeError('conv2d: input has %d channels, weight expects %d' % (ci, ci2))
+    return _shape(n, 2 * h, 2 * w, ci, co, r, s, 1, pad, 2 * h + 2 * pad - r + 1, 2 * w + 2 * pad - s + 1)
+
+
+def up_conv_fused(x, weight, pad):
+    if not (UP_FUSE and x.dim() == 4 and x.is_cuda and x.dtype == torch.float32 and not _prefix[0]):
+        return False
+    shp = _up_conv_shape(x, weight, pad)
+    return query('xas_conv_up2_fused', shp, 0) == 1 and query('xas_conv_up2_fused', shp, 2) == 1
+
+
+class _UpConv2d(torch.autograd.Function):
+
+    @staticmethod
+    def forward(ctx, x, weight, bias, pad, cache):
+        x = to_cl(x)
+        n, ci, h, w = x.shape
+        shp, x_slot = with_act_amax(_up_conv_shape(x, weight, pad), x)
+        y = empty_cl(n, shp.Cout, shp.Ho, shp.Wo, x)
+        call('xas_conv_fwd', ptr(x), ptr(cache.get(weight, 0, shp)), ptr(bias), ptr(y), _x_up2(shp))
+        up_stats['fused'] += 1
+        ctx.save_for_backward(x, weight, *([bias] if bias is not None else []))
+        ctx.shp, ctx.cache, ctx.has_bias, ctx.x_slot = shp, cache, bias is not None, x_slot
+        if ctx.needs_input_grad[1]:
+            note_use(weight)
+        if bias is not None and ctx.needs_input_grad[2]:
+            note_use(bias)
+        return y
+
+    @staticmethod
+    def backward(ctx, dy):
+        x, weight, *rest = ctx.saved_tensors
+        shp = with_grad_amax(ctx.shp, dy, ctx.x_slot)
+        dy = to_cl(dy)
+        n, ci, h, w = x.shape
+        dx = dw = db = None
+        if ctx.needs_input_grad[0]:
+            du = empty_cl(n, ci, 2 * h, 2 * w, dy)
+            call('xas_conv_dgrad', ptr(dy), ptr(ctx.cache.get(weight, 1, shp)), ptr(du), shp)
+            dx = empty_cl(n, ci, h, w, dy)
+            call('xas_upsample2x_bwd', ptr(du), n, h, w, ci, ptr(dx))
+        shp_w = _x_up2(shp)
+        if ctx.needs_input_grad[1] and not _wgrad_into_grad(x, dy, shp_w, weight):
+            dw = _wgrad(x, dy, shp_w, weight.shape)
+        if ctx.has_bias and ctx.needs_input_grad[2]:
+            M = shp.N * shp.Ho * shp.Wo
+            if not _bias_into_grad(dy, M, shp.Cout, rest[0]):
+                db = _bias_grad(dy, M, shp.Cout)
+        return dx, dw, db, None, None
+
+
+def upsample2x_conv2d(x, weight, bias, pad, cache):
+    if up_conv_fused(x, weight, pad):
+        return _UpConv2d.apply(x, weight, bias, pad, cache)
+    up_stats['separate'] += 1
+    return conv2d(upsample2x(x), weight, bias, 1, pad, cache)
+
+
 class _Sigmoid(torch.autograd.Function):
     @staticmethod
     def forward(ctx, x):
diff --git a/x-as-supervision_amd/xas_amd/prof.py b/x-as-supervision_amd/xas_amd/prof.py
--- a/x-as-supervision_amd/xas_amd/prof.py
+++ b/x-as-supervision_amd/xas_amd/prof.py
@@ -37,8 +37,8 @@
 
 
 def conv_bytes(shape):
-    return 4.0 * (shape.N * shape.Hi * shape.Wi * shape.Cin + shape.Cout * shape.R * shape.S * shape.Cin
-                  + shape.N * shape.Ho * shape.Wo * shape.Cout)
+    x_pixels = shape.N * shape.Hi * shape.Wi // (4 if shape.mode & 0x200 else 1)
+    return 4.0 * (x_pixels * shape.Cin + shape.Cout * shape.R * shape.S * shape.Cin + shape.N * shape.Ho * shape.Wo * shape.Cout)
 
 
 class KernelTimer:
```

After: 2112 images/s (median of 6 runs). No clear change (+0.2%).
